# langtech-bsc/quantool

Hardware: AMD Instinct MI355X
Metric: quantized weights/sec (GPTQ int4, Llama-3-8B, 512 calib samples) (higher is better)
Workload: dtype f32

## Files before the change

### include/quantool_amd.h

```cpp
#ifndef QUANTOOL_AMD_H
#define QUANTOOL_AMD_H

#include <stddef.h>
#include <stdint.h>

#ifdef __cplusplus
extern "C" {
#endif

typedef void* qt_stream_t;

enum qt_status {
    QT_OK = 0,
    QT_ERR_INVALID = -1,
    QT_ERR_NOT_PD = -2,
    QT_ERR_WORKSPACE = -3,
    QT_ERR_HIP = -4,
    QT_ERR_UNSUPPORTED = -5
};

enum qt_dtype { QT_F32 = 0, QT_BF16 = 1, QT_F16 = 2 };

int qt_version(void);
const char* qt_last_error(void);

size_t qt_xtx_workspace_bytes(int64_t n_tokens, int K);
int qt_xtx_accumulate(const void* X, int x_dtype, int64_t n_tokens, int K, int64_t ldx, float* G,
                      void* workspace, size_t workspace_bytes, qt_stream_t stream);

int qt_xtx_accumulate_batched(const void* const* X, int x_dtype, const int64_t* n_tokens, const int64_t* ldx, int K,
                              float* const* G, int n_problems, void* workspace, size_t workspace_bytes,
                              qt_stream_t stream);
int qt_xtx_batched_plan(const int64_t* n_tokens, int n_problems, int K, int32_t* items, int max_items, int* n_items,
                        int* n_slabs, size_t* workspace_bytes);

size_t qt_xtx_accumulate_f32_workspace_bytes(int64_t n_tokens, int K);
int qt_xtx_accumulate_f32(const float* X, int64_t n_tokens, int K, int64_t ldx, float* G, void* workspace,
                          size_t workspace_bytes, qt_stream_t stream);

size_t qt_act_stats_workspace_bytes(int64_t n_tokens, int K);
int qt_act_stats_accumulate(const void* X, int x_dtype, int64_t n_tokens, int K, int64_t ldx, float* abs_sum,
                            float* cmin, float* cmax, void* workspace, size_t workspace_bytes,
                            qt_stream_t stream);

size_t qt_hessian_prepare_workspace_bytes(int K);
int qt_hessian_prepare(const float* G, int K, int64_t n_samples, float percdamp,
                       const int32_t* perm, float* A, uint8_t* dead, float* diag_out,
                       void* workspace, size_t workspace_bytes, qt_stream_t stream);
int qt_hessian_prepare_damp(const float* G, int K, int64_t n_samples, float percdamp,
                            const int32_t* perm, float* A, uint8_t* dead, float* diag_out, float* damp_out,
                            void* workspace, size_t workspace_bytes, qt_stream_t stream);
int qt_hessian_diag(const float* G, int K, int64_t n_samples, float* diag_out, qt_stream_t stream);
int qt_argsort_desc(const float* values, int K, int32_t* perm, int32_t* inv, qt_stream_t stream);

size_t qt_cholesky_inverse_upper_workspace_bytes(int K);
int qt_cholesky_inverse_upper(float* A, int K, float* U, int32_t* info, void* workspace,
                              size_t workspace_bytes, qt_stream_t stream);

size_t qt_cholesky_inverse_upper_batched_workspace_bytes(int K, int n_problems);
int qt_cholesky_inverse_upper_batched(float* A, int64_t strideA, int K, float* U, int64_t strideU, int32_t* info,
                                      int n_problems, void* workspace, size_t workspace_bytes, qt_stream_t stream);

int qt_cholesky_inverse_upper_bounded(float* A, int K, float* U, int32_t* info, const float* min_eig_lb,
                                      void* workspace, size_t workspace_bytes, qt_stream_t stream);
int qt_cholesky_inverse_upper_batched_bounded(float* A, int64_t strideA, int K, float* U, int64_t strideU, int32_t* info,
                                              int n_problems, const float* min_eig_lb, void* workspace,
                                              size_t workspace_bytes, qt_stream_t stream);

int qt_group_minmax_qparams(const void* W, int w_dtype, int R, int K, int64_t ldw, int group_size,
                            int symmetric, int num_bits, float* scale, float* zp, float* scale_t,
                            float* zp_t, qt_stream_t stream);

int qt_weight_gather_f32(const void* W, int w_dtype, int R, int K, int64_t ldw, const int32_t* perm,
                         const uint8_t* dead, float* W_f32, qt_stream_t stream);

int qt_weight_gather_qparams(const void* W, int w_dtype, int R, int K, int64_t ldw, const int32_t* perm,
                             const uint8_t* dead, int group_size, int symmetric, int num_bits, float* W_f32, float* scale,
                             float* zp, float* scale_t, float* zp_t, int64_t ld_t, qt_stream_t stream);

size_t qt_gptq_sweep_workspace_bytes(int R, int K, int blocksize);
int qt_gptq_sweep(float* W, int R, int K, const float* U, const float* scale_t, const float* zp_t,
                  int G, const int32_t* g_idx, int blocksize, int num_bits, int8_t* Qt,
                  float* loss, void* workspace, size_t workspace_bytes, qt_stream_t stream);

int qt_gptq_sweep_grouped(float* W, int R, int K, const float* U, int64_t strideU, int n_groups, const int32_t* row_end,
                          const float* scale_t, const float* zp_t, int G, const int32_t* g_idx, int blocksize,
                          int num_bits, int8_t* Qt, float* loss, void* workspace, size_t workspace_bytes,
                          qt_stream_t stream);

int qt_pack_int4(const int8_t* Qt, int R, int K, const int32_t* col_src, int32_t* packed,
                 qt_stream_t stream);

int qt_dequantize(const int8_t* Qt, int R, int K, const int32_t* col_src, const float* scale,
                  const float* zp, int G, const int32_t* g_of_col, void* out, int out_dtype,
                  int64_t ldo, qt_stream_t stream);

size_t qt_awq_weight_mean_workspace_bytes(int R, int K);
int qt_awq_weight_mean_accumulate(const void* W, int w_dtype, int R, int K, int64_t ldw, int group_size,
                                  float* w_sum, void* workspace, size_t workspace_bytes,
                                  qt_stream_t stream);
int qt_awq_scales(const float* x_abs_sum, int64_t n_tokens, const float* w_sum, int64_t n_rows, int K,
                  int n_grid, int duo_scaling, float* scales, qt_stream_t stream);
int qt_symmetrize_lower(float* G, int K, qt_stream_t stream);
size_t qt_awq_loss_workspace_bytes(int R, int K);
int qt_awq_loss(const void* W, int w_dtype, int R, int K, int64_t ldw, const float* s, int group_size,
                int symmetric, int num_bits, const float* Gfull, int64_t n_tokens, int exact, float weight,
                int accumulate, float* loss_out, void* workspace, size_t workspace_bytes, qt_stream_t stream);
size_t qt_awq_losses_workspace_bytes(int R, int K, int n_grid);
int qt_awq_losses(const void* W, int w_dtype, int R, int K, int64_t ldw, const float* scales, int n_grid,
                  int group_size, int symmetric, int num_bits, const float* Gfull, int64_t n_tokens, float weight,
                  int accumulate, float* losses, void* workspace, size_t workspace_bytes, qt_stream_t stream);
int qt_argmin_f32(const float* values, int n, int32_t* index_out, qt_stream_t stream);
int qt_awq_pseudo_quantize(const void* W, int w_dtype, int R, int K, int64_t ldw, const float* s, int group_size,
                           int symmetric, int num_bits, void* out, int64_t ldo, qt_stream_t stream);
int qt_scale_columns(const void* W, int w_dtype, int R, int K, int64_t ldw, const float* s, int divide,
                     void* out, int64_t ldo, qt_stream_t stream);
int qt_rtn_quantize(const void* W, int w_dtype, int R, int K, int64_t ldw, const float* scale,
                    const float* zp, int G, int group_size, int num_bits, int8_t* Qt, qt_stream_t stream);

size_t qt_col_absmax_workspace_bytes(int R, int K);
int qt_col_absmax_accumulate(const void* W, int w_dtype, int R, int K, int64_t ldw, float* wmax,
                             void* workspace, size_t workspace_bytes, qt_stream_t stream);
int qt_smoothquant_scales(const float* cmin, const float* cmax, const float* wmax, int K, float alpha,
                          float* s, qt_stream_t stream);

size_t qt_sgemm_tn_f32_workspace_bytes(int M, int N);
int qt_sgemm_tn_f32(const float* A, int64_t lda, const float* B, int64_t ldb, const float* Cin,
                    int64_t ldcin, float* Cout, int64_t ldcout, int M, int N, int kdim, int skip_zero_k,
                    int mode, int allow_split_k, void* workspace, size_t workspace_bytes, qt_stream_t stream);

int qt_xtx_tile_table_check(int K, int* n_tiles_out, int* chunk_panels_out, int* round_panels_out);

size_t qt_xtx_dot_workspace_bytes(int64_t n_tokens, int K);
int qt_xtx_dot(const void* X, int x_dtype, int64_t n_tokens, int K, int64_t ldx, const float* H, double scale,
               float* out, int accumulate, void* workspace, size_t workspace_bytes, qt_stream_t stream);

size_t qt_gemm3_tn_f32_workspace_bytes(int M, int N, int k);
int qt_gemm3_tn_f32(const float* A, int64_t lda, const float* B, int64_t ldb, float* C, int64_t ldc, int M,
                    int N, int k, int kind, void* workspace, size_t workspace_bytes, qt_stream_t stream);
int qt_gemm3_tn_f32_ex(const float* A, int64_t lda, const float* B, int64_t ldb, float* C, int64_t ldc, int M, int N,
                       int k, int kind, int tri, int tight, int batch, int64_t bsA, int64_t bsB, int64_t bsC,
                       void* workspace, size_t workspace_bytes, qt_stream_t stream);

int qt_gemm3_tn_f16x2(const float* A, int64_t lda, const float* B, int64_t ldb, float* C, int64_t ldc, int M, int N,
                      int k, int kind, int tri, int tight, int batch, int64_t bsA, int64_t bsB, int64_t bsC,
                      const float* bound_a, const float* bound_b, void* workspace, size_t workspace_bytes,
                      qt_stream_t stream);

int qt_gemm3_plan_check(int Tm, int Tn, int c_end, int tri, int* n_items_out, int* n_slabs_out, int* longest_out);
int qt_chol_g3_plan_check(int K, int merged, int min_chunks, long long* counts_out);
enum qt_act { QT_ACT_SILU = 0 };
#define QT_I8_MID_MAX_M 128
#define QT_I8_MID_K_UNIT 128
#define QT_I8_RING_K_UNIT 128
#define QT_I8_RING_SLOTS 8
#define QT_I8_RING_LEAD 6
#define QT_I8_RING_W4_K_UNIT 128
#define QT_I8_RING_W4_SLOTS 8
#define QT_I8_RING_W4_LEAD 6
#define QT_SPLITK_I8_K_UNIT 128
#define QT_SPLITK_I8_MAX_SPLITS 32
#define QT_SPLITK_I8_MIN_K_TILES 4
#define QT_MOE_I8_WIDE_K_UNIT 128
#define QT_MOE_I8_WIDE_TILE_ROWS 128
#define QT_MOE_I8_WIDE_MAX_E 4096
enum qt_weight_format { QT_W_INT8 = 0, QT_W_INT4_PACKED = 1 };
int qt_quantize_tokens_i8(const void* X, int x_dtype, int64_t M, int K, int64_t ldx, const int32_t* col_perm,
                          int symmetric, int8_t* Xq, float* s_x, int32_t* zp_x, qt_stream_t stream);
int qt_act_mul_quantize_i8(const void* gate, int64_t ldg, const void* up, int64_t ldu, int x_dtype, int64_t M, int K,
                           int act, const int32_t* col_perm, int symmetric, int8_t* Xq, float* s_x, int32_t* zp_x,
                           void* H, int64_t ldh, qt_stream_t stream);
int qt_rmsnorm_quantize_i8(const void* X, int64_t ldx, const void* weight, int x_dtype, int64_t M, int K, float eps,
                           const int32_t* col_perm, int symmetric, int8_t* Xq, float* s_x, int32_t* zp_x,
                           void* Y, int64_t ldy, float* rstd, qt_stream_t stream);
int qt_gemm_i8(const int8_t* Xq, int64_t M, int K, const void* Wq, int w_format, int N, const float* s_x,
               const int32_t* zp_x, const float* s_w, int G, const int32_t* wsum, const void* bias, void* Y,
               int out_dtype, int64_t ldy, qt_stream_t stream);
int qt_gemm_i8_skinny(const int8_t* Xq, int M, int K, const void* Wq, int w_format, int N, const float* s_x,
                      const int32_t* zp_x, const float* s_w, int G, const int32_t* wsum, const void* bias, void* Y,
                      int out_dtype, int64_t ldy, qt_stream_t stream);
int qt_gemm_i8_ring(const int8_t* Xq, int64_t M, int K, const void* Wq, int w_format, int N, const float* s_x,
                    const int32_t* zp_x, const float* s_w, int G, const int32_t* wsum, const void* bias, void* Y,
                    int out_dtype, int64_t ldy, qt_stream_t stream);
int qt_gemm_i8_ring_w4(const int8_t* Xq, int64_t M, int K, const void* Wq, int w_format, int N, const float* s_x,
                       const int32_t* zp_x, const float* s_w, int G, const int32_t* wsum, const void* bias, void* Y,
                       int out_dtype, int64_t ldy, qt_stream_t stream);
int qt_gemm_i8_mid(const int8_t* Xq, int64_t M, int K, const void* Wq, int w_format, int N, const float* s_x,
                   const int32_t* zp_x, const float* s_w, int G, const int32_t* wsum, const void* bias, void* Y,
                   int out_dtype, int64_t ldy, qt_stream_t stream);
int qt_splitk_gemm_i8_plan(int64_t M, int N, int K, int cus, int splits_requested, int* splits,
                           size_t* workspace_size);
int qt_splitk_gemm_i8_range(int k_tiles, int splits, int s, int* t0, int* t1);
int qt_splitk_gemm_i8(const int8_t* Xq, int64_t M, int K, const void* Wq, int w_format, int N, const float* s_x,
                      const int32_t* zp_x, const float* s_w, int G, const int32_t* wsum, const void* bias, void* Y,
                      int out_dtype, int64_t ldy, int splits, void* workspace, size_t workspace_size,
                      qt_stream_t stream);

int qt_moe_route(const void* top_k_index, int index_is_int64, int64_t T, int k, int E, int32_t* offsets,
                 int32_t* src_token, int32_t* src_slot, int32_t* row_of, qt_stream_t stream);
int qt_gemm_i8_grouped(const int8_t* Xq, int K, const int32_t* row_idx, int64_t R, const int32_t* offsets, int E,
                       const void* Wq, int w_format, int N, const float* s_x, const int32_t* zp_x, const float* s_w,
                       int G, const int32_t* wsum, void* Y, int out_dtype, int64_t ldy, qt_stream_t stream);
int qt_gemm_i8_skinny_grouped(const int8_t* Xq, int K, const int32_t* row_idx, int64_t R, const int32_t* offsets,
                              int E, const void* Wq, int w_format, int N, const float* s_x, const int32_t* zp_x,
                              const float* s_w, int G, const int32_t* wsum, void* Y, int out_dtype, int64_t ldy,
                              qt_stream_t stream);
int qt_gemm_i8_ring_grouped(const int8_t* Xq, int K, const int32_t* row_idx, int64_t R, const int32_t* offsets, int E,
                            const void* Wq, int w_format, int N, const float* s_x, const int32_t* zp_x,
                            const float* s_w, int G, const int32_t* wsum, void* Y, int out_dtype, int64_t ldy,
                            int64_t x_rows, qt_stream_t stream);
int qt_moe_gemm_i8_ring_w4(const int8_t* Xq, int K, const int32_t* row_idx, int64_t R, const int32_t* offsets, int E,
                           const void* Wq, int w_format, int N, const float* s_x, const int32_t* zp_x,
                           const float* s_w, int G, const int32_t* wsum, void* Y, int out_dtype, int64_t ldy,
                           int64_t x_rows, qt_stream_t stream);
int qt_moe_gemm_i8_wide(const int8_t* Xq, int K, const int32_t* row_idx, int64_t R, const int32_t* offsets, int E,
                        const void* Wq, int w_format, int N, const float* s_x, const int32_t* zp_x, const float* s_w,
                        int G, const int32_t* wsum, void* Y, int out_dtype, int64_t ldy, int64_t x_rows,
                        qt_stream_t stream);
int qt_moe_combine(const void* Y, int dtype, int H, int64_t ldy, const int32_t* row_of, const float* weights,
                   int64_t T, int k, void* out, qt_stream_t stream);

int qt_dequantize_weight(const void* Wq, int w_format, int N, int K, const float* s_w, int G, const int8_t* zp_w,
                         const int32_t* g_idx, void* W, int dtype, int64_t ldw, qt_stream_t stream);
int qt_gemm_wq_skinny(const void* X, int x_dtype, int M, int K, int64_t ldx, const void* Wq, int w_format, int N,
                      const float* s_w, int G, const int8_t* zp_w, const int32_t* g_idx, const void* bias, void* Y,
                      int64_t ldy, qt_stream_t stream);

int qt_gemm_wq_stream(const void* X, int x_dtype, int M, int K, int64_t ldx, const void* Wq, int w_format, int N,
                      const float* s_w, int G, const int8_t* zp_w, const int32_t* g_idx, const void* bias, void* Y,
                      int64_t ldy, qt_stream_t stream);
#define QT_WQ_STREAM_MAX_M 128
#define QT_WQ_STREAM_K_UNIT 128
#define QT_WQ_STREAM_MAX_LDX 33554432
// ... 36 lines not shown
```

### quantool_amd/csrc/cholesky.hip

```cpp
#include <stdlib.h>
#include <string.h>

#include <map>
#include <tuple>
#include <vector>

#include "chol_layout.h"
#include "common.h"
#include "gemm3_tn.h"
#include "sgemm_tn.h"

namespace {

static_assert(CHOL_CHUNK_ROWS == G3_CHUNK_ROWS, "chol_layout.h counts k chunks as gemm3_tn.h cuts them");
static int chol_block_env(const char* name) {
    const char* e = getenv(name);
    if (!e) return 0;
    int x = atoi(e) / 128 * 128;
    return x < 128 ? 128 : (x > NBO_MAX ? NBO_MAX : x);
}
struct G3Step {
    int n_items = 0, n_red = 0;
    size_t item_off = 0, red_off = 0;
};
// ... 448 lines not shown
    const int blk = blk0 + blockIdx.x;
    const int n = (K - blk * NB < NB) ? K - blk * NB : NB;
    const float* Rd = Rd_all + (size_t)blk * RD_STRIDE;
    const int tid = threadIdx.x, lane = tid & 63, wave = tid >> 6;
    {
        constexpr int NV = RD_STRIDE / 4 / 256;
        f32x4 v[NV];
#pragma unroll
        for (int r = 0; r < NV; ++r) v[r] = ((const f32x4*)Rd)[tid + 256 * r];
#pragma unroll
        for (int r = 0; r < NV; ++r) ((f32x4*)Rs)[tid + 256 * r] = v[r];
    }
    const float* D32 = Rs + NB * NB;
    const int l31 = lane & 31, h = lane >> 5;
    const int col = wave * 32 + l31;

    f32x16 acc[4];
#pragma unroll
    for (int a = 0; a < 4; ++a)
#pragma unroll
        for (int r = 0; r < 16; ++r) {
            const int row = 32 * a + (r & 3) + 8 * (r >> 2) + 4 * h;
            acc[a][r] = (row == col) ? 1.0f : 0.0f;
        }
    __syncthreads();

#pragma unroll
    for (int b = 0; b < 4; ++b) {
        f32x16 zb;
#pragma unroll
        for (int r = 0; r < 16; ++r) zb[r] = 0.0f;
#pragma unroll
        for (int r = 0; r < 16; ++r) {
            const int k = (r & 3) + 8 * (r >> 2) + 4 * h;
            const float av = D32[(b * 32 + k) * 32 + l31];
            zb = __builtin_amdgcn_mfma_f32_32x32x2f32(av, acc[b][r], zb, 0, 0, 0);
        }
        acc[b] = zb;
#pragma unroll
        for (int a = b + 1; a < 4; ++a) {
#pragma unroll
            for (int r = 0; r < 16; ++r) {
                const int k = (r & 3) + 8 * (r >> 2) + 4 * h;
                const float av = -Rs[(32 * b + k) * NB + 32 * a + l31];
                acc[a] = __builtin_amdgcn_mfma_f32_32x32x2f32(av, zb[r], acc[a], 0, 0, 0);
            }
        }
    }
    float* Dinv = Dinv_all + (size_t)blk * NB * NB;
    float* Yd = Y + (size_t)(blk * NB) * ldy + blk * NB;
#pragma unroll
    for (int a = 0; a < 4; ++a)
#pragma unroll
        for (int r = 0; r < 16; ++r) {
            const int row = 32 * a + (r & 3) + 8 * (r >> 2) + 4 * h;
            const bool in = row < n && col < n;
            const float z = (in && row >= col) ? acc[a][r] : 0.0f;
            Dinv[col * NB + row] = z;
            if (in) Yd[(size_t)row * ldy + col] = z;
        }
}

__global__ __launch_bounds__(256) void transpose_lower_block_kernel(const float* __restrict__ Y, int64_t ldy, int w,
                                                                    float* __restrict__ XT, int ldx, int64_t bsY,
                                                                    int64_t bsXT) {
    if (blockIdx.z) {
        Y += (size_t)blockIdx.z * bsY;
        XT += (size_t)blockIdx.z * bsXT;
    }
    __shared__ float tile[32][33];
    const int bx = blockIdx.x * 32, by = blockIdx.y * 32;
    const int tx = threadIdx.x & 31, ty = threadIdx.x >> 5;
    for (int r = ty; r < 32; r += 8) {
        const int m = bx + r, k = by + tx;
        tile[r][tx] = (m < w && k < w && k <= m) ? Y[(size_t)m * ldy + k] : 0.0f;
    }
    __syncthreads();
    for (int r = ty; r < 32; r += 8) {
        const int k = by + r, m = bx + tx;
        if (k < w && m < w) XT[(size_t)k * ldx + m] = tile[tx][r];
    }
}

__global__ __launch_bounds__(256) void flat_reverse_lower_to_upper_kernel(float* __restrict__ U, int K, int64_t bsU) {
    U += (size_t)blockIdx.z * bsU;
    const int j = blockIdx.x * blockDim.x + threadIdx.x;
    const int i = blockIdx.y;
    if (j >= K || j < i) return;
    const size_t e = (size_t)i * K + j;
    const size_t pe = (size_t)(K - 1 - i) * K + (K - 1 - j);
    if (i == j) {
        if (e <= pe) {
            const float t = U[e];
            U[e] = U[pe];
            U[pe] = t;
        }
    } else {
        U[e] = U[pe];
        U[pe] = 0.0f;
    }
}

__global__ __launch_bounds__(256) void identity_if_failed_kernel(float* __restrict__ U, int K,
                                                                 const int32_t* __restrict__ info, int64_t bsU) {
    if (info[blockIdx.z] == 0) return;
    U += (size_t)blockIdx.z * bsU;
    for (int i = blockIdx.x; i < K; i += gridDim.x)
        for (int j = threadIdx.x; j < K; j += blockDim.x) U[(size_t)i * K + j] = (i == j) ? 1.0f : 0.0f;
}

__global__ __launch_bounds__(256) void chol_scales_kernel(const float* __restrict__ A, int64_t bsA, int K,
                                                          const float* __restrict__ min_eig_lb, int32_t* __restrict__ e,
                                                          int32_t* __restrict__ info) {
    __shared__ float red[256];
    const int b = blockIdx.x, nprob = gridDim.x;
    const float* Ab = A + (size_t)b * bsA;
    float m = 0.0f;
    for (int i = threadIdx.x; i < K; i += 256) m = fmaxf(m, Ab[(size_t)i * K + i]);
    red[threadIdx.x] = m;
    __syncthreads();
    for (int s = 128; s > 0; s >>= 1) {
        if ((int)threadIdx.x < s) red[threadIdx.x] = fmaxf(red[threadIdx.x], red[threadIdx.x + s]);
        __syncthreads();
    }
    if (threadIdx.x == 0) {
        auto clampe = [](float t) { return (int)fminf(fmaxf(t, (float)-G3_E_MAX), (float)G3_E_MAX); };
        const float d = red[0], lb = min_eig_lb[b];
        e[b] = (d > 0.0f && d < 3.0e38f) ? clampe(3.0f - ceilf(0.5f * log2f(d))) : 0;
        if (lb > 0.0f && lb < 3.0e38f) {
            e[nprob + b] = clampe(3.0f - ceilf(-0.5f * log2f(lb)));
        } else {
            e[nprob + b] = 0;
            info[b] = K + 1;
        }
    }
}

}


static CholLayout chol_layout(int K, const CholG3Plan* g3) { return CholLayout(K, g3->any, g3->max_slabs); }

extern "C" size_t qt_cholesky_inverse_upper_batched_workspace_bytes(int K, int n_problems) {
    if (K <= 0 || n_problems <= 0) return 0;
    int nbo_, nbi_;
    const CholG3Plan* g3 = chol_blocks(K, nbo_, nbi_);
    return chol_layout(K, g3).batch_bytes(n_problems, g3->blob_bytes);
}

extern "C" size_t qt_cholesky_inverse_upper_workspace_bytes(int K) {
    return qt_cholesky_inverse_upper_batched_workspace_bytes(K, 1);
}

constexpr size_t INV_LDS = (size_t)(NB * LDT + NB * LDP) * sizeof(float);
constexpr size_t POTF2_LDS = (size_t)(NB * LDA + 4 * 32 * 32) * sizeof(float);
constexpr size_t RD_LDS = RD_STRIDE * sizeof(float);

struct CholCtx {
    float *A, *Y;
    int K, nprob, NBO, NBI;
    int64_t sA, sY, sW;
    float *T, *TI, *XT, *Rd, *Dinv, *split_ws;
    size_t split_ws_bytes;
    unsigned short *Rpl, *Ypl;
    int64_t plane_stride;
    float* g3_slabs;
    char* g3_tab;
    const CholG3Plan* g3;
    const CholG3Plan* tab;
    int planes;
    int merge_mode;
    int32_t *info, *eR, *eY;
    int prio;
    hipStream_t stream;
};

static int chol_resolve(CholCtx& c, const float* min_eig_lb) {
    bool f16x2 = min_eig_lb != nullptr;
    if (const char* e = getenv("QT_CHOL_PLANES")) {
        if (strcmp(e, "bf16x3") == 0) f16x2 = false;
        else if (strcmp(e, "f16x2") == 0) {
            QT_CHECK_ARG(min_eig_lb, "qt_cholesky_inverse_upper: QT_CHOL_PLANES=f16x2 needs a bound on lambda_min (the _bounded entry points)");
        } else {
// ... 166 lines not shown
    if (rc) return rc;
    return split_row(c, I);
}

static int chol_run_two_phase(const CholCtx& c) {
    for (BlockRow J(c.K, c.NBO); J; ++J) {
        int rc = fac_product(c, J);
        if (!rc) rc = fac_panels(c, J);
        if (rc) return rc;
    }
    int rc = trinv(c, 0, (c.K + NB - 1) / NB);
    if (rc) return rc;
    for (BlockRow I(c.K, c.NBI); I; ++I) {
        rc = inv_product(c, I);
        if (!rc) rc = inv_row(c, I);
        if (rc) return rc;
    }
    return QT_OK;
}

static int chol_run_walk(const CholCtx& c) {
    for (BlockRow J(c.K, c.NBO); J; ++J) {
        int rc;
        if (c.merge_mode == CHOL_WALK_MERGED && c.tab->row[J.Jb].n_items > 0) {
            rc = g3_row(c, c.tab->row[J.Jb], c.Rpl, J.J0, J.J0, J.rows(), c.K - J.J0, c.A + (size_t)J.J0 * c.K + J.J0, IN_A, G3_SUB,
                        true);
        } else {
            rc = fac_product(c, J);
            if (!rc) rc = inv_product(c, J);
        }
        if (!rc) rc = fac_panels(c, J);
        if (!rc) rc = trinv(c, J.J0 / NB, (J.rows() + NB - 1) / NB);
        if (!rc) rc = inv_row(c, J);
        if (rc) return rc;
    }
    return QT_OK;
}

static hipError_t chol_lds_attrs() {
    static QtOncePerDevice lds_attr;
    return lds_attr.run([] {
        const auto attr = hipFuncAttributeMaxDynamicSharedMemorySize;
        hipError_t e = hipFuncSetAttribute((const void*)potf2_kernel, attr, (int)POTF2_LDS);
        if (e == hipSuccess) e = hipFuncSetAttribute((const void*)trsm_rt_kernel, attr, (int)RD_LDS);
        if (e == hipSuccess) e = hipFuncSetAttribute((const void*)trinv_batched_kernel, attr, (int)INV_LDS);
        if (e == hipSuccess) e = hipFuncSetAttribute((const void*)trinv_mfma_kernel, attr, (int)RD_LDS);
        return e;
    });
}

static int chol_run(float* A, int64_t strideA, int K, float* U, int64_t strideU, int32_t* info, int nprob, void* workspace,
                    size_t workspace_bytes, hipStream_t stream, const float* min_eig_lb = nullptr) {
    CholCtx c = {};
    c.A = A; c.Y = U; c.K = K; c.nprob = nprob; c.info = info; c.stream = stream;
    if (int rc = chol_resolve(c, min_eig_lb)) return rc;
    const CholLayout L = chol_layout(K, c.g3);
    const size_t need = L.batch_bytes(nprob, c.g3->blob_bytes);
    if (!workspace || workspace_bytes < need) {
        qt_set_error("qt_cholesky_inverse_upper: workspace %zu < required %zu", workspace_bytes, need);
        return QT_ERR_WORKSPACE;
    }
    char* ws = (char*)qt_align_up((size_t)workspace, 256);
    c.sW = (int64_t)(L.bytes() / 4); c.sA = nprob > 1 ? strideA : 0; c.sY = nprob > 1 ? strideU : 0;
    c.T = (float*)(ws + L.T); c.TI = (float*)(ws + L.TI); c.XT = (float*)(ws + L.XT);
    c.Rd = (float*)(ws + L.Rd); c.Dinv = (float*)(ws + L.Dinv);
    c.split_ws = (float*)(ws + L.split); c.split_ws_bytes = L.split_bytes;
    c.plane_stride = (int64_t)K * K;
    if (c.g3->any) {
        c.Rpl = (unsigned short*)(ws + L.Rpl); c.Ypl = (unsigned short*)(ws + L.Ypl);
        c.g3_slabs = (float*)(ws + L.slabs); c.g3_tab = ws + L.tables(nprob);
        QT_HIP(hipMemcpyAsync(c.g3_tab, c.tab->blob, c.tab->blob_bytes, hipMemcpyHostToDevice, stream));
    }
    static_assert(2 * SG_MAX_BATCH * sizeof(int32_t) <= (size_t)NB * NB * 2, "the exponents fit the smallest third plane");
    c.eR = c.planes == G3_F16X2 ? (int32_t*)(c.Rpl + 2 * c.plane_stride) : nullptr;
    c.eY = c.planes == G3_F16X2 ? c.eR + nprob : nullptr;
    QT_HIP(chol_lds_attrs());
    QT_HIP(hipMemsetAsync(info, 0, sizeof(int32_t) * nprob, stream));
    c.prio = qt_chain_prio();
    if (c.planes == G3_F16X2) {
        hipLaunchKernelGGL(chol_scales_kernel, dim3(nprob), dim3(256), 0, stream, (const float*)A, c.sA, K, min_eig_lb, c.eR, info);
        QT_LAUNCH_CHECK();
    }
    if (int rc = c.merge_mode == CHOL_TWO_PHASE ? chol_run_two_phase(c) : chol_run_walk(c)) return rc;
    hipLaunchKernelGGL(flat_reverse_lower_to_upper_kernel, dim3((K + 255) / 256, K, nprob), dim3(256), 0, stream, U, K, c.sY);
    QT_LAUNCH_CHECK();
    hipLaunchKernelGGL(identity_if_failed_kernel, dim3(K < 1024 ? K : 1024, 1, nprob), dim3(256), 0, stream, U, K,
                       (const int32_t*)info, c.sY);
    QT_LAUNCH_CHECK();
    return QT_OK;
}

static int chol_check_batch(const char* fn, bool ptrs, int K, int n_problems, int64_t strideA, int64_t strideU) {
    QT_CHECK_ARG(K > 0 && ptrs && n_problems >= 1 && n_problems <= SG_MAX_BATCH, "%s: bad arguments (1 <= n_problems <= %d)", fn,
                 SG_MAX_BATCH);
    QT_CHECK_ARG(n_problems == 1 || (strideA >= (int64_t)K * K && strideU >= (int64_t)K * K && strideA % 4 == 0 && strideU % 4 == 0),
                 "%s: strides must be multiples of 4 elements and >= K*K", fn);
    return QT_OK;
}

extern "C" int qt_cholesky_inverse_upper(float* A, int K, float* U, int32_t* info, void* workspace,
                                         size_t workspace_bytes, qt_stream_t stream_) {
    QT_CHECK_ARG(K > 0 && A && U && info, "qt_cholesky_inverse_upper: bad arguments");
    return chol_run(A, 0, K, U, 0, info, 1, workspace, workspace_bytes, (hipStream_t)stream_);
}

extern "C" int qt_cholesky_inverse_upper_batched(float* A, int64_t strideA, int K, float* U, int64_t strideU, int32_t* info,
                                                 int n_problems, void* workspace, size_t workspace_bytes,
                                                 qt_stream_t stream_) {
    if (int rc = chol_check_batch("qt_cholesky_inverse_upper_batched", A && U && info, K, n_problems, strideA, strideU)) return rc;
    return chol_run(A, strideA, K, U, strideU, info, n_problems, workspace, workspace_bytes, (hipStream_t)stream_);
}

extern "C" int qt_cholesky_inverse_upper_bounded(float* A, int K, float* U, int32_t* info, const float* min_eig_lb,
                                                 void* workspace, size_t workspace_bytes, qt_stream_t stream_) {
    QT_CHECK_ARG(K > 0 && A && U && info && min_eig_lb, "qt_cholesky_inverse_upper_bounded: bad arguments");
    return chol_run(A, 0, K, U, 0, info, 1, workspace, workspace_bytes, (hipStream_t)stream_, min_eig_lb);
}

extern "C" int qt_cholesky_inverse_upper_batched_bounded(float* A, int64_t strideA, int K, float* U, int64_t strideU,
                                                         int32_t* info, int n_problems, const float* min_eig_lb,
                                                         void* workspace, size_t workspace_bytes, qt_stream_t stream_) {
    if (int rc = chol_check_batch("qt_cholesky_inverse_upper_batched_bounded", A && U && info && min_eig_lb, K, n_problems,
                                  strideA, strideU))
        return rc;
    return chol_run(A, strideA, K, U, strideU, info, n_problems, workspace, workspace_bytes, (hipStream_t)stream_, min_eig_lb);
}

extern "C" int qt_chol_g3_plan_check(int K, int merged, int min_chunks, long long* counts_out) {
    if (K <= 0) return -1;
    constexpr int NBX = 512, TRI_STEP = 256 / G3_CHUNK_ROWS;
    if (min_chunks <= 0) min_chunks = 64;
    const int cap = chol_g3_target_items(K);
    CholG3Plan sep, pl;
    std::vector<char> sep_bytes, bytes;
    chol_g3_build(K, NBX, NBX, min_chunks, cap, false, sep, sep_bytes);
    chol_g3_build(K, NBX, NBX, min_chunks, cap, merged != 0, pl, bytes);
    if (pl.max_slabs > sep.max_slabs || pl.blob_bytes > sep.blob_bytes) return -2;
    long long launches = 0, n_items = 0, n_slabs = 0;
    auto check = [&](const G3Step& st, int Tm, int Tn0, int tri0, int Tn1, int c_end) -> int {
        if (st.n_items <= 0) return 0;
        const G3Item* items = (const G3Item*)(bytes.data() + st.item_off);
        const G3Red* red = (const G3Red*)(bytes.data() + st.red_off);
        if (st.n_items > cap && st.n_items > Tm * (Tn0 + Tn1)) return -3;
        const int Tn[2] = {Tn0, Tn1};
        auto lo_of = [&](int seg, int tj) { return (seg == 1 || tri0) ? TRI_STEP * tj : 0; };
        std::vector<int> cover((size_t)2 * Tm * (Tn0 + Tn1 + 1) * c_end, 0);
        auto cell = [&](int seg, int ti, int tj, int c) { return (((size_t)seg * Tm + ti) * (Tn0 + Tn1 + 1) + tj) * c_end + c; };
        std::vector<int> owner(sep.max_slabs, -1);
        int slabs_here = 0;
        for (int q = 0; q < st.n_items; ++q) {
            const G3Item& it = items[q];
            const int seg = (it.tile & G3_SEG_BIT) ? 1 : 0, ti = it.tile >> 16, tj = it.tile & G3_TJ_MASK;
            if (ti < 0 || ti >= Tm || tj >= Tn[seg]) return -4;
            const int lo = lo_of(seg, tj);
            if (it.c_lo < lo || it.c_hi > c_end || it.c_hi - it.c_lo < 2) return -5;
            for (int c = it.c_lo; c < it.c_hi; ++c) cover[cell(seg, ti, tj, c)]++;
            if (it.slab < 0) {
                if (it.c_lo != lo || it.c_hi != c_end) return -6;
            } else {
                if (it.slab >= sep.max_slabs) return -7;
                if (owner[it.slab] >= 0) return -8;
                owner[it.slab] = q;
                ++slabs_here;
            }
        }
        for (int seg = 0; seg < 2; ++seg)
            for (int ti = 0; ti < Tm; ++ti)
                for (int tj = 0; tj < Tn[seg]; ++tj)
                    for (int c = 0; c < c_end; ++c)
                        if (cover[cell(seg, ti, tj, c)] != (c >= lo_of(seg, tj) ? 1 : 0)) return -9;
        int in_red = 0;
        for (int r = 0; r < st.n_red; ++r) {
            const G3Red& e = red[r];
            if (e.count < 2 || e.first < 0 || e.first + e.count > sep.max_slabs || (e.seg != 0 && e.seg != 1)) return -10;
            const int want_tile = e.tile | (e.seg ? G3_SEG_BIT : 0);
            int prev_hi = lo_of(e.seg, e.tile & G3_TJ_MASK);
            for (int q = 0; q < e.count; ++q) {
                const int o = owner[e.first + q];
                if (o < 0 || items[o].tile != want_tile || items[o].c_lo != prev_hi) return -11;
                prev_hi = items[o].c_hi;
// ... 33 lines not shown
```

### quantool_amd/csrc/quant.hip

```cpp
#include "common.h"

namespace {


__device__ __forceinline__ float wave_min(float v) {
#pragma unroll
    for (int o = 32; o > 0; o >>= 1) v = fminf(v, __shfl_xor(v, o));
    return v;
}
__device__ __forceinline__ float wave_max(float v) {
#pragma unroll
    for (int o = 32; o > 0; o >>= 1) v = fmaxf(v, __shfl_xor(v, o));
    return v;
}

__global__ __launch_bounds__(64) void qparams_kernel(const void* __restrict__ W, int dtype, int R, int K,
                                                     int64_t ldw, int gs, int symmetric, float qmin, float qmax,
                                                     float* __restrict__ scale, float* __restrict__ zp,
                                                     float* __restrict__ scale_t, float* __restrict__ zp_t) {
    const int g = blockIdx.x, r = blockIdx.y, lane = threadIdx.x;
    const int G = K / gs;
    const size_t base = (size_t)r * ldw + (size_t)g * gs;
    float mn = INFINITY, mx = -INFINITY;
    for (int c = lane; c < gs; c += 64) {
        const float w = qt_load_w(W, dtype, base + c);
        mn = fminf(mn, w);
        mx = fmaxf(mx, w);
    }
    mn = wave_min(mn);
    mx = wave_max(mx);
    if (lane == 0) {
        mn = fminf(mn, 0.0f);
        mx = fmaxf(mx, 0.0f);
        float s, z;
        const float eps = 1.1920928955078125e-07f;
        if (symmetric) {
            const float amax = fmaxf(fabsf(mn), fabsf(mx));
            s = amax / ((qmax - qmin) / 2.0f);
            s = fmaxf(s, eps);
            z = 0.0f;
        } else {
            s = (mx - mn) / (qmax - qmin);
            s = fmaxf(s, eps);
            z = qmin - mn / s;
            z = fminf(fmaxf(rintf(z), qmin), qmax);
        }
        scale[(size_t)r * G + g] = s;
        zp[(size_t)r * G + g] = z;
        if (scale_t) scale_t[(size_t)g * R + r] = s;
        if (zp_t) zp_t[(size_t)g * R + r] = z;
    }
}

__global__ __launch_bounds__(256) void gather_f32_kernel(const void* __restrict__ W, int dtype, int R, int K,
                                                         int64_t ldw, const int32_t* __restrict__ perm,
                                                         const uint8_t* __restrict__ dead, float* __restrict__ out) {
    const int s = blockIdx.x * blockDim.x + threadIdx.x;
    const int r = blockIdx.y;
    if (s >= K) return;
    const int src = perm ? perm[s] : s;
    float v = qt_load_w(W, dtype, (size_t)r * ldw + src);
    if (dead && dead[s]) v = 0.0f;
    out[(size_t)r * K + s] = v;
}

template <typename T>
__global__ __launch_bounds__(256) void gather_qparams_kernel(const T* __restrict__ W, int dtype, int R, int K, int64_t ldw,
                                                             const int32_t* __restrict__ perm,
                                                             const uint8_t* __restrict__ dead, int gs, int symmetric,
                                                             float qmin, float qmax, float* __restrict__ out,
                                                             float* __restrict__ scale, float* __restrict__ zp,
                                                             float* __restrict__ scale_t, float* __restrict__ zp_t,
                                                             int64_t ld_t) {
    extern __shared__ __attribute__((aligned(16))) unsigned char smem[];
    T* row = (T*)smem;
    const int r = blockIdx.x, tid = threadIdx.x, lane = tid & 63, wave = tid >> 6;
    const T* src = W + (size_t)r * ldw;
    constexpr int V = 16 / sizeof(T);
    if ((((uintptr_t)src) & 15) == 0 && K % V == 0) {
        for (int c = tid * V; c < K; c += 256 * V) *(f32x4*)(row + c) = *(const f32x4*)(src + c);
    } else {
        for (int c = tid; c < K; c += 256) row[c] = src[c];
// ... 41 lines not shown
            f32x4 v;
#pragma unroll
            for (int e = 0; e < 4; ++e) {
                const int sp = s4 + e;
                const float x = val(perm ? perm[sp] : sp);
                v[e] = (dead && dead[sp]) ? 0.0f : x;
            }
            *(f32x4*)(dst + s4) = v;
        }
    } else {
        for (int sp = tid; sp < K; sp += 256) {
            const float x = val(perm ? perm[sp] : sp);
            dst[sp] = (dead && dead[sp]) ? 0.0f : x;
        }
    }
}

__global__ __launch_bounds__(256) void pack_int4_kernel(const int8_t* __restrict__ Qt, int R, int K,
                                                        const int32_t* __restrict__ col_src,
                                                        int32_t* __restrict__ packed) {
    __shared__ uint32_t tile[64][33];
    const int Kw = (K + 7) / 8;
    const int r0 = blockIdx.y * 64, w0 = blockIdx.x * 32;
    const int tid = threadIdx.x;
    for (int e = tid; e < 64 * 32; e += 256) {
        const int rl = e & 63, wl = e >> 6;
        const int r = r0 + rl, w = w0 + wl;
        uint32_t acc = 0;
        if (r < R && w < Kw) {
#pragma unroll
            for (int j = 0; j < 8; ++j) {
                const int c = w * 8 + j;
                if (c < K) {
                    const int sc = col_src ? col_src[c] : c;
                    const uint32_t u = ((uint32_t)((int)Qt[(size_t)sc * R + r] + 8)) & 0xFu;
                    acc |= u << (4 * j);
                }
            }
        }
        tile[rl][wl] = acc;
    }
    __syncthreads();
    for (int e = tid; e < 64 * 32; e += 256) {
        const int wl = e & 31, rl = e >> 5;
        const int r = r0 + rl, w = w0 + wl;
        if (r < R && w < Kw) packed[(size_t)r * Kw + w] = (int32_t)tile[rl][wl];
    }
}

__global__ __launch_bounds__(256) void pack_int4_rows4_kernel(const int8_t* __restrict__ Qt, int R, int K,
                                                              const int32_t* __restrict__ col_src,
                                                              int32_t* __restrict__ packed) {
    __shared__ uint32_t tile[256][33];
    const int Kw = (K + 7) / 8;
    const int r0 = blockIdx.y * 256, w0 = blockIdx.x * 32;
    const int tid = threadIdx.x;
    for (int e = tid; e < 64 * 32; e += 256) {
        const int rq = e & 63, wl = e >> 6;
        const int r = r0 + 4 * rq, w = w0 + wl;
        uint32_t acc[4] = {0, 0, 0, 0};
        if (r < R && w < Kw) {
#pragma unroll
            for (int j = 0; j < 8; ++j) {
                const int c = w * 8 + j;
                if (c < K) {
                    const int sc = col_src ? col_src[c] : c;
                    const uint32_t q4 = *(const uint32_t*)(Qt + (size_t)sc * R + r);
#pragma unroll
                    for (int i = 0; i < 4; ++i) {
                        const uint32_t u = (uint32_t)((int)(int8_t)(q4 >> (8 * i)) + 8) & 0xFu;
                        acc[i] |= u << (4 * j);
                    }
                }
            }
        }
#pragma unroll
        for (int i = 0; i < 4; ++i) tile[4 * rq + i][wl] = acc[i];
    }
    __syncthreads();
    for (int e = tid; e < 256 * 32; e += 256) {
        const int wl = e & 31, rl = e >> 5;
        const int r = r0 + rl, w = w0 + wl;
        if (r < R && w < Kw) packed[(size_t)r * Kw + w] = (int32_t)tile[rl][wl];
    }
}

__global__ __launch_bounds__(256) void dequant_kernel(const int8_t* __restrict__ Qt, int R, int K,
                                                      const int32_t* __restrict__ col_src,
                                                      const float* __restrict__ scale, const float* __restrict__ zp,
                                                      int G, const int32_t* __restrict__ g_of_col,
                                                      void* __restrict__ out, int out_dtype, int64_t ldo) {
    __shared__ float tile[64][65];
    const int r0 = blockIdx.y * 64, c0 = blockIdx.x * 64;
    const int tid = threadIdx.x;
    for (int e = tid; e < 64 * 64; e += 256) {
        const int rl = e & 63, cl = e >> 6;
        const int r = r0 + rl, c = c0 + cl;
        float v = 0.0f;
        if (r < R && c < K) {
            const int sc = col_src ? col_src[c] : c;
            v = (float)Qt[(size_t)sc * R + r];
        }
        tile[rl][cl] = v;
    }
    __syncthreads();
    for (int e = tid; e < 64 * 64; e += 256) {
        const int cl = e & 63, rl = e >> 6;
        const int r = r0 + rl, c = c0 + cl;
        if (r < R && c < K) {
            const int g = g_of_col[c];
            const float q = tile[rl][cl];
            const float z = zp[(size_t)r * G + g];
            const float v = (q - z) * scale[(size_t)r * G + g];
            qt_store_w(out, out_dtype, (size_t)r * ldo + c, v);
        }
    }
}

}

static inline void qt_range(int num_bits, float* qmin, float* qmax) {
    *qmin = -(float)(1 << (num_bits - 1));
    *qmax = (float)((1 << (num_bits - 1)) - 1);
}

extern "C" int qt_group_minmax_qparams(const void* W, int w_dtype, int R, int K, int64_t ldw, int group_size,
                                       int symmetric, int num_bits, float* scale, float* zp, float* scale_t,
                                       float* zp_t, qt_stream_t stream_) {
    hipStream_t stream = (hipStream_t)stream_;
    QT_CHECK_ARG(W && scale && zp && R > 0 && K > 0, "qt_group_minmax_qparams: bad arguments");
    QT_CHECK_ARG(qt_dtype_ok(w_dtype), "qt_group_minmax_qparams: dtype %d unsupported", w_dtype);
    QT_CHECK_ARG(num_bits >= 2 && num_bits <= 8, "qt_group_minmax_qparams: num_bits=%d", num_bits);
    const int gs = group_size <= 0 ? K : group_size;
    QT_CHECK_ARG(K % gs == 0, "qt_group_minmax_qparams: K=%d not divisible by group_size=%d", K, gs);
    float qmin, qmax;
    qt_range(num_bits, &qmin, &qmax);
    const size_t esz = qt_dtype_size(w_dtype);
    const int G = K / gs;
    for (int row0 = 0; row0 < R; row0 += 32768) {
        const int rows = (R - row0 < 32768) ? R - row0 : 32768;
        hipLaunchKernelGGL(qparams_kernel, dim3(G, rows), dim3(64), 0, stream,
                           (const void*)((const char*)W + (size_t)row0 * ldw * esz), w_dtype, R, K, ldw, gs, symmetric,
                           qmin, qmax, scale + (size_t)row0 * G, zp + (size_t)row0 * G,
                           scale_t ? scale_t + row0 : nullptr, zp_t ? zp_t + row0 : nullptr);
        QT_LAUNCH_CHECK();
    }
    return QT_OK;
}

extern "C" int qt_weight_gather_f32(const void* W, int w_dtype, int R, int K, int64_t ldw, const int32_t* perm,
                                    const uint8_t* dead, float* W_f32, qt_stream_t stream_) {
    hipStream_t stream = (hipStream_t)stream_;
    QT_CHECK_ARG(W && W_f32 && R > 0 && K > 0, "qt_weight_gather_f32: bad arguments");
    QT_CHECK_ARG(qt_dtype_ok(w_dtype), "qt_weight_gather_f32: dtype %d unsupported", w_dtype);
    const size_t esz = qt_dtype_size(w_dtype);
    for (int row0 = 0; row0 < R; row0 += 32768) {
        const int rows = (R - row0 < 32768) ? R - row0 : 32768;
        hipLaunchKernelGGL(gather_f32_kernel, dim3((K + 255) / 256, rows), dim3(256), 0, stream,
                           (const void*)((const char*)W + (size_t)row0 * ldw * esz), w_dtype, rows, K, ldw, perm, dead,
                           W_f32 + (size_t)row0 * K);
        QT_LAUNCH_CHECK();
    }
    return QT_OK;
}

extern "C" int qt_weight_gather_qparams(const void* W, int w_dtype, int R, int K, int64_t ldw, const int32_t* perm,
                                        const uint8_t* dead, int group_size, int symmetric, int num_bits, float* W_f32,
                                        float* scale, float* zp, float* scale_t, float* zp_t, int64_t ld_t,
                                        qt_stream_t stream_) {
    hipStream_t stream = (hipStream_t)stream_;
    QT_CHECK_ARG(W && W_f32 && scale && zp && R > 0 && K > 0, "qt_weight_gather_qparams: bad arguments");
    QT_CHECK_ARG(qt_dtype_ok(w_dtype), "qt_weight_gather_qparams: dtype %d unsupported", w_dtype);
    QT_CHECK_ARG(num_bits >= 2 && num_bits <= 8, "qt_weight_gather_qparams: num_bits=%d", num_bits);
    const int gs = group_size <= 0 ? K : group_size;
    QT_CHECK_ARG(K % gs == 0, "qt_weight_gather_qparams: K=%d not divisible by group_size=%d", K, gs);
    QT_CHECK_ARG((!scale_t && !zp_t) || ld_t >= R, "qt_weight_gather_qparams: ld_t=%lld < R=%d", (long long)ld_t, R);
    const size_t esz = qt_dtype_size(w_dtype);
    const size_t lds = qt_align_up((size_t)K * esz, 16);
    QT_CHECK_ARG(lds <= 160 * 1024, "qt_weight_gather_qparams: a row of %d elements does not fit the LDS", K);
    QT_CHECK_ARG(((uintptr_t)W_f32 & 15) == 0, "qt_weight_gather_qparams: W_f32 must be 16-byte aligned");
    float qmin, qmax;
    qt_range(num_bits, &qmin, &qmax);
    static QtOncePerDevice attr16, attr32;
    if (esz == 2) {
        QT_HIP(attr16.run([&] {
            return hipFuncSetAttribute((const void*)gather_qparams_kernel<unsigned short>,
                                       hipFuncAttributeMaxDynamicSharedMemorySize, 160 * 1024);
        }));
        hipLaunchKernelGGL(gather_qparams_kernel<unsigned short>, dim3(R), dim3(256), lds, stream, (const unsigned short*)W,
                           w_dtype, R, K, ldw, perm, dead, gs, symmetric, qmin, qmax, W_f32, scale, zp, scale_t, zp_t, ld_t);
    } else {
        QT_HIP(attr32.run([&] {
            return hipFuncSetAttribute((const void*)gather_qparams_kernel<float>, hipFuncAttributeMaxDynamicSharedMemorySize,
                                       160 * 1024);
        }));
        hipLaunchKernelGGL(gather_qparams_kernel<float>, dim3(R), dim3(256), lds, stream, (const float*)W, w_dtype, R, K, ldw,
                           perm, dead, gs, symmetric, qmin, qmax, W_f32, scale, zp, scale_t, zp_t, ld_t);
    }
    QT_LAUNCH_CHECK();
    return QT_OK;
}

extern "C" int qt_pack_int4(const int8_t* Qt, int R, int K, const int32_t* col_src, int32_t* packed,
                            qt_stream_t stream_) {
    hipStream_t stream = (hipStream_t)stream_;
    QT_CHECK_ARG(Qt && packed && R > 0 && K > 0, "qt_pack_int4: bad arguments");
    const int Kw = (K + 7) / 8;
    if (R % 4 == 0 && (((uintptr_t)Qt) & 3) == 0 && (R + 255) / 256 <= 65535)
        hipLaunchKernelGGL(pack_int4_rows4_kernel, dim3((Kw + 31) / 32, (R + 255) / 256), dim3(256), 0, stream, Qt, R, K,
                           col_src, packed);
    else
        hipLaunchKernelGGL(pack_int4_kernel, dim3((Kw + 31) / 32, (R + 63) / 64), dim3(256), 0, stream, Qt, R, K, col_src,
                           packed);
    QT_LAUNCH_CHECK();
    return QT_OK;
}

extern "C" int qt_dequantize(const int8_t* Qt, int R, int K, const int32_t* col_src, const float* scale,
                             const float* zp, int G, const int32_t* g_of_col, void* out, int out_dtype, int64_t ldo,
                             qt_stream_t stream_) {
    hipStream_t stream = (hipStream_t)stream_;
    QT_CHECK_ARG(Qt && scale && zp && g_of_col && out && R > 0 && K > 0 && G > 0, "qt_dequantize: bad arguments");
    QT_CHECK_ARG(qt_dtype_ok(out_dtype), "qt_dequantize: dtype %d unsupported", out_dtype);
    hipLaunchKernelGGL(dequant_kernel, dim3((K + 63) / 64, (R + 63) / 64), dim3(256), 0, stream, Qt, R, K, col_src,
                       scale, zp, G, g_of_col, out, out_dtype, ldo);
    QT_LAUNCH_CHECK();
    return QT_OK;
}
```

### quantool_amd/csrc/xtx.hip

```cpp
#include <stdlib.h>
#include <string.h>

#include <algorithm>
#include <map>
#include <type_traits>
#include <vector>

#include "common.h"
#include "ring_pipe.h"

namespace {

constexpr int BKT = 64;
constexpr int RING = 8;

struct XtxParams {
    const void* X;
    const void* tail;
    int64_t ldx;
    int K;
    int n_tt;
    int has_tail;
    const int* tile_tab;
    int n_direct;
    int n_rem;
    int s2;
    float* slabs;
    float* G;
    int map_mode;
    int wrap_units;
    unsigned* progress;
    int thr_win;
    int thr_nap;
    int thr_chk;
    const float* H;
    double* dot_partials;
    int batch_items;
    int64_t x_batch_bytes;
    const struct XtxBItem* b_items;
    const struct XtxBProb* b_probs;
};

struct XtxBItem {
    int prob;
    int tile;
    int tt0, cnt;
    int slab;
    int pad[3];
};
struct XtxBProb {
    const void* X;
    const void* tail;
    float* G;
    int64_t ldx;
    int n_tt, has_tail;
    int64_t pad[3];
};
struct XtxBRed {
    int prob, tile, slab0, n_chunks, stride;
    int pad[3];
};
static_assert(sizeof(XtxBItem) == 32 && sizeof(XtxBProb) == 64 && sizeof(XtxBRed) == 32, "table records");

__device__ __forceinline__ int xtx_uni(int v) { return __builtin_amdgcn_readfirstlane(v); }
__device__ __forceinline__ uint64_t xtx_uni64(uint64_t v) {
    const unsigned lo = (unsigned)__builtin_amdgcn_readfirstlane((int)(unsigned)v);
    const unsigned hi = (unsigned)__builtin_amdgcn_readfirstlane((int)(unsigned)(v >> 32));
    return ((uint64_t)hi << 32) | lo;
}

__device__ __forceinline__ int xtx_logical(int map_mode) {
    const int b = blockIdx.x, nwg = gridDim.x;
    if (map_mode != 0) return b;
    const int round = b >> 8, rb = b & 255;
    const int m = min(256, nwg - (round << 8));
    const int xcd = rb & 7, idx = rb >> 3, q8 = m >> 3, r8 = m & 7;
    return (round << 8) + (xcd < r8 ? xcd * (q8 + 1) : r8 * (q8 + 1) + (xcd - r8) * q8) + idx;
}

__device__ __forceinline__ int xtx_item(const XtxParams& p, int logical, int& tt0, int& cnt, int& slab_idx) {
    int tile_idx;
    slab_idx = -1;
    if (logical < p.n_direct) {
        tile_idx = logical;
        tt0 = 0;
        cnt = p.n_tt;
    } else {
        const int l2 = logical - p.n_direct;
        const int chunk = l2 / p.n_rem;
        tile_idx = p.n_direct + (l2 - chunk * p.n_rem);
        const int base_cnt = p.n_tt / p.s2, rem = p.n_tt % p.s2;
        tt0 = chunk * base_cnt + (chunk < rem ? chunk : rem);
        cnt = base_cnt + (chunk < rem ? 1 : 0);
        slab_idx = l2;
    }
    return p.tile_tab[tile_idx];
}


template <bool WRAP, bool F16, bool THROTTLE>
__global__ __launch_bounds__(NTHREADS, 2) void xtx_kernel(XtxParams p) {
    constexpr int LEAD = 6;
    __shared__ __attribute__((aligned(16))) char ring[RING * UNIT_BYTES + (THROTTLE ? 1024 : 0)];
    const int tid = threadIdx.x;
    const int lane = tid & 63;
    const int wave = __builtin_amdgcn_readfirstlane(tid >> 6);
    const int wave_m = wave >> 2, wave_n = wave & 3;
    const bool group_b = wave >= 4;

    const int logical = xtx_logical(p.map_mode);
    int tt0, cnt, slab_idx;
    const int tt_packed = xtx_item(p, logical, tt0, cnt, slab_idx);
    const int ti = tt_packed >> 16, tj = tt_packed & 0xFFFF;
    const int nu = cnt * (BKT / UT);
    const int K = p.K;
    const size_t ld2 = (size_t)p.ldx * 2;

    const int rsub = lane >> 4;
    const int lch = (lane & 15) ^ (rsub << 2);
    const int trow = 4 * (wave & 3) + rsub;
    int colA = ti * BT + (wave >> 2) * 128 + lch * 8;
    int colB = tj * BT + (wave >> 2) * 128 + lch * 8;
    colA = colA > K - 8 ? K - 8 : colA;
    colB = colB > K - 8 ? K - 8 : colB;
// ... 73 lines not shown
    const int rowpart = (8 * (g >> 1) + q) * 256 + 32 * (g & 1) + 8 * pp;
    int aoff[4], boff[2];
#pragma unroll
    for (int mi = 0; mi < 4; ++mi) aoff[mi] = wave_m * 4096 + rowpart + 64 * (mi ^ q);
#pragma unroll
    for (int ni = 0; ni < 2; ++ni)
        boff[ni] = (2 + (wave_n >> 1)) * 4096 + rowpart + 64 * ((((wave_n & 1) << 1) + ni) ^ q);

    f32x16 acc[4][2];
#pragma unroll
    for (int mi = 0; mi < 4; ++mi)
#pragma unroll
        for (int ni = 0; ni < 2; ++ni)
#pragma unroll
            for (int r = 0; r < 16; ++r) acc[mi][ni][r] = 0.0f;

    s16x8 fa[4], fb[2];
    auto drain_wait = [&](int u) {
        ring_drain_wait<2, LEAD>(nu - u - 2);
    };
    auto phase = [&](auto slot_c, auto steady_c, int u) {
        constexpr int S = decltype(slot_c)::value;
        constexpr bool STEADY = decltype(steady_c)::value;
        constexpr int ISLOT = (S + LEAD) & (RING - 1);
        const char* base = ring + S * UNIT_BYTES;
#pragma unroll
        for (int mi = 0; mi < 4; ++mi) fa[mi] = tr_load8(base + aoff[mi]);
#ifdef QT_XTX_ABL_LDS
        fb[0] = tr_load8(base + boff[0]);
        fb[1] = fb[0];
#else
#pragma unroll
        for (int ni = 0; ni < 2; ++ni) fb[ni] = tr_load8(base + boff[ni]);
#endif
        if (STEADY) {
            issue_running(ISLOT);
            wait_vmcnt<2 * (LEAD - 1)>();
        } else if (u + LEAD < nu) {
            issue(u + LEAD, ISLOT);
            wait_vmcnt<2 * (LEAD - 1)>();
        } else {
            drain_wait(u);
        }
#ifdef QT_XTX_ABL_HALF
        constexpr int MI_N = 2;
#else
        constexpr int MI_N = 4;
#endif
        ring_sync_math([&] { ring_mma32<F16, MI_N>(fa, fb, acc); });
    };
    auto body8 = [&](auto steady_c, int u) {
        if (THROTTLE && throttled && (u & (p.thr_chk - 1)) == 0) throttle_step(u);
        ring_body<8>([&](auto slot_c, int uu) { phase(slot_c, steady_c, uu); }, u);
    };

    if (nu > 0) {
#pragma unroll
        for (int i = 0; i < LEAD; ++i)
            if (i < nu) issue(i, i);
        if (nu >= LEAD) wait_vmcnt<2 * (LEAD - 1)>();
        else wait_vmcnt<0>();
        ring_stagger_begin(group_b);

        const int steady_end = (nu < i_tail ? nu : i_tail);
        run_src += (size_t)LEAD * ustride;
        int u = 0;
        for (; u + 8 + LEAD <= steady_end; u += 8) body8(std::true_type{}, u);
        for (; u + 8 <= nu; u += 8) body8(std::false_type{}, u);
        if (u < nu) {
            phase(std::integral_constant<int, 0>{}, std::false_type{}, u);
            phase(std::integral_constant<int, 1>{}, std::false_type{}, u + 1);
            phase(std::integral_constant<int, 2>{}, std::false_type{}, u + 2);
            phase(std::integral_constant<int, 3>{}, std::false_type{}, u + 3);
        }
        ring_stagger_end(group_b);
        if (THROTTLE && throttled && lane == 0) {
            unsigned* dst = prog_round + prog_member;
            const unsigned val = 0x7fffffffu;
            asm volatile("global_store_dword %0, %1, off sc0 sc1\n\ts_nop 1" ::"v"(dst), "v"(val) : "memory");
        }
    }

    const int jl = lane & 31, ih = 4 * (lane >> 5);
    if (slab_idx < 0) {
#pragma unroll
        for (int mi = 0; mi < 4; ++mi)
#pragma unroll
            for (int ni = 0; ni < 2; ++ni) {
                const int gj = tj * BT + wave_n * 64 + ni * 32 + jl;
#pragma unroll
                for (int r = 0; r < 16; ++r) {
                    const int gi = ti * BT + wave_m * 128 + mi * 32 + (r & 3) + 8 * (r >> 2) + ih;
                    if (gi < K && gj < K) {
                        float* dst = p.G + (size_t)gi * K + gj;
                        *dst = *dst + acc[mi][ni][r];
                    }
                }
            }
    } else {
        float* slab = p.slabs + (size_t)slab_idx * (size_t)(BT * BT);
#pragma unroll
        for (int mi = 0; mi < 4; ++mi)
#pragma unroll
            for (int ni = 0; ni < 2; ++ni)
#pragma unroll
                for (int r = 0; r < 16; ++r) {
                    const int i_loc = wave_m * 128 + mi * 32 + (r & 3) + 8 * (r >> 2) + ih;
                    const int j_loc = wave_n * 64 + ni * 32 + jl;
                    slab[i_loc * BT + j_loc] = acc[mi][ni][r];
                }
    }
}

constexpr int RING16 = 10;
constexpr int DBL_BYTES = 2 * UNIT_BYTES;

template <bool F16, bool DOT = false, bool BATCHED = false>
__global__ __launch_bounds__(NTHREADS, 2) void xtx16_kernel(XtxParams p) {
    static_assert(!(DOT && BATCHED), "the fused product has its own batch form");
    constexpr int ND = 5;
    constexpr int LEAD = 3;
    __shared__ __attribute__((aligned(16))) char ring[RING16 * UNIT_BYTES];
    const int tid = threadIdx.x;
    const int lane = tid & 63;
    const int wave = __builtin_amdgcn_readfirstlane(tid >> 6);
    const int wave_m = wave >> 2, wave_n = wave & 3;
    const bool group_b = wave >= 4;

    int logical = xtx_logical(p.map_mode);
    const int item_global = logical;
    const char* Xb = (const char*)p.X;
    if (DOT) {
        const int prob = logical / p.batch_items;
        logical -= prob * p.batch_items;
        Xb += (size_t)prob * (size_t)p.x_batch_bytes;
    }
    int tt0, cnt, slab_idx, tt_packed;
    const void* tailp = p.tail;
    float* Gp = p.G;
    int64_t ldx = p.ldx;
    int n_tt = p.n_tt, has_tail = p.has_tail;
    if (BATCHED) {
        const XtxBItem* it = p.b_items + logical;
        const XtxBProb* pr = p.b_probs + xtx_uni(it->prob);
        tt_packed = xtx_uni(it->tile);
        tt0 = xtx_uni(it->tt0);
        cnt = xtx_uni(it->cnt);
        slab_idx = xtx_uni(it->slab);
        Xb = (const char*)xtx_uni64((uint64_t)pr->X);
        tailp = (const void*)xtx_uni64((uint64_t)pr->tail);
        Gp = (float*)xtx_uni64((uint64_t)pr->G);
        ldx = (int64_t)xtx_uni64((uint64_t)pr->ldx);
        n_tt = xtx_uni(pr->n_tt);
        has_tail = xtx_uni(pr->has_tail);
    } else {
        tt_packed = xtx_item(p, logical, tt0, cnt, slab_idx);
    }
    const int ti = tt_packed >> 16, tj = tt_packed & 0xFFFF;
    const int nd = cnt * (BKT / (2 * UT));
    const int K = p.K;
    const size_t ld2 = (size_t)ldx * 2;

    const int rsub = lane >> 4;
    const int row_hi = (wave & 3) >> 1;
    const int lch = (lane & 15) ^ (rsub << 2) ^ (row_hi << 1);
    const int trow = 4 * (wave & 3) + rsub;
    int colA = ti * BT + (wave >> 2) * 128 + lch * 8;
// ... 36 lines not shown
        for (int bj = 0; bj < 4; ++bj)
#pragma unroll
            for (int r = 0; r < 4; ++r) acc[ai][bj][r] = 0.0f;

    s16x8 fa[8], fb[4];
    auto drain_wait = [&](int d) {
        ring_drain_wait<4, LEAD>(nd - d - 2);
    };
    auto phase = [&](auto slot_c, auto steady_c, int d) {
        constexpr int S = decltype(slot_c)::value;
        constexpr bool STEADY = decltype(steady_c)::value;
        constexpr int ISLOT = (S + LEAD) % ND;
        const char* base = ring + S * DBL_BYTES;
#pragma unroll
        for (int ai = 0; ai < 8; ++ai) fa[ai] = tr_load8(base + aoff[ai]);
#pragma unroll
        for (int bj = 0; bj < 4; ++bj) fb[bj] = tr_load8(base + boff[bj]);
        if (STEADY) {
            issue_at(run_src, ISLOT);
            run_src += 2 * ustride;
            wait_vmcnt<4 * (LEAD - 1)>();
        } else if (d + LEAD < nd) {
            issue_at(dbl_src(d + LEAD), ISLOT);
            wait_vmcnt<4 * (LEAD - 1)>();
        } else {
            drain_wait(d);
        }
        ring_sync_math([&] { ring_mma16<F16>(fa, fb, acc); });
    };

    if (nd > 0) {
#pragma unroll
        for (int i = 0; i < LEAD; ++i)
            if (i < nd) issue_at(dbl_src(i), i);
        if (nd >= LEAD) wait_vmcnt<4 * (LEAD - 1)>();
        else wait_vmcnt<0>();
        ring_stagger_begin(group_b);

        const int steady_end = (nd < d_tail ? nd : d_tail);
        run_src += (size_t)LEAD * 2 * ustride;
        int d = 0;
        for (; d + ND + LEAD <= steady_end; d += ND)
            ring_body<ND>([&](auto slot_c, int dd) { phase(slot_c, std::true_type{}, dd); }, d);
        for (; d < nd; d += ND) {
            phase(std::integral_constant<int, 0>{}, std::false_type{}, d);
            if (d + 1 < nd) phase(std::integral_constant<int, 1>{}, std::false_type{}, d + 1);
            if (d + 2 < nd) phase(std::integral_constant<int, 2>{}, std::false_type{}, d + 2);
            if (d + 3 < nd) phase(std::integral_constant<int, 3>{}, std::false_type{}, d + 3);
            if (d + 4 < nd) phase(std::integral_constant<int, 4>{}, std::false_type{}, d + 4);
        }
        ring_stagger_end(group_b);
    }

    const int jl = lane & 15, ih = 4 * (lane >> 4);
    if (DOT) {
        double part = 0.0;
#pragma unroll
        for (int ai = 0; ai < 8; ++ai)
#pragma unroll
            for (int bj = 0; bj < 4; ++bj) {
                const int gj = tj * BT + wave_n * 64 + bj * 16 + jl;
#pragma unroll
                for (int r = 0; r < 4; ++r) {
                    const int gi = ti * BT + wave_m * 128 + ai * 16 + ih + r;
                    if (gi < K && gj <= gi) {
                        const double v = (double)p.H[(size_t)gi * K + gj] * (double)acc[ai][bj][r];
                        part += (gj < gi) ? 2.0 * v : v;
                    }
                }
            }
#pragma unroll
        for (int off = 32; off > 0; off >>= 1) part += __shfl_xor(part, off);
        double* red = (double*)ring;
        if (lane == 0) red[wave] = part;
        __syncthreads();
        if (tid == 0) {
            double t = red[0];
#pragma unroll
            for (int w = 1; w < 8; ++w) t += red[w];
            p.dot_partials[item_global] = t;
        }
        return;
    }
    if (slab_idx < 0) {
#pragma unroll
        for (int ai = 0; ai < 8; ++ai)
#pragma unroll
            for (int bj = 0; bj < 4; ++bj) {
                const int gj = tj * BT + wave_n * 64 + bj * 16 + jl;
#pragma unroll
                for (int r = 0; r < 4; ++r) {
                    const int gi = ti * BT + wave_m * 128 + ai * 16 + ih + r;
                    if (gi < K && gj < K) {
                        float* dst = Gp + (size_t)gi * K + gj;
                        *dst = *dst + acc[ai][bj][r];
                    }
                }
            }
    } else {
        float* slab = p.slabs + (size_t)slab_idx * (size_t)(BT * BT);
#pragma unroll
        for (int ai = 0; ai < 8; ++ai)
#pragma unroll
            for (int bj = 0; bj < 4; ++bj)
#pragma unroll
                for (int r = 0; r < 4; ++r) {
                    const int i_loc = wave_m * 128 + ai * 16 + ih + r;
                    const int j_loc = wave_n * 64 + bj * 16 + jl;
                    slab[i_loc * BT + j_loc] = acc[ai][bj][r];
                }
    }
}

__global__ __launch_bounds__(256) void xtx_reduce_kernel(const float* __restrict__ slabs, int n_rem, int n_splits,
                                                         float* __restrict__ G, int K,
                                                         const int* __restrict__ tile_tab) {
    const int tile = blockIdx.x;
    const int tt_packed = tile_tab[tile];
    const int ti = tt_packed >> 16, tj = tt_packed & 0xFFFF;
    const int part = blockIdx.y;
    const size_t tile_elems = (size_t)BT * BT;
    for (int e = threadIdx.x; e < 16 * (BT / 4); e += blockDim.x) {
        const int i_loc = part * 16 + e / (BT / 4);
        const int j_loc = (e % (BT / 4)) * 4;
        const int gi = ti * BT + i_loc, gj = tj * BT + j_loc;
        if (gi >= K || gj >= K) continue;
        f32x4 s = {0.f, 0.f, 0.f, 0.f};
        for (int sp = 0; sp < n_splits; ++sp) {
            const f32x4 v = *(const f32x4*)(slabs + ((size_t)sp * n_rem + tile) * tile_elems +
                                            (size_t)i_loc * BT + j_loc);
            s += v;
        }
        float* dst = G + (size_t)gi * K + gj;
        if (gj + 3 < K) {
            f32x4 o = *(f32x4*)dst;
            o += s;
            *(f32x4*)dst = o;
        } else {
            for (int c = 0; c < 4 && gj + c < K; ++c) dst[c] += s[c];
        }
    }
}

struct XtxPlan {
    int n_tiles, n_tt, has_tail;
    int n_direct, n_rem, s2;
    size_t slab_bytes, tail_bytes, tab_bytes, prog_bytes;
};

static void xtx_tile_order_pairs(int nt, std::vector<int>& tab) {
    const int m = 8, nb = (nt + m - 1) / m;
    auto blk = [&](int a, int b) {
        const int r0 = a * m, r1 = std::min(nt, r0 + m), c0 = b * m, c1 = std::min(nt, c0 + m);
        if (a == b) {
            for (int ti = r0; ti < r1; ++ti)
                for (int tj = c0; tj <= ti; ++tj) tab.push_back((ti << 16) | tj);
        } else {
            for (int si = r0; si < r1; si += 4)
                for (int ti = si; ti < std::min(si + 4, r1); ++ti)
                    for (int tj = c0; tj < c1; ++tj) tab.push_back((ti << 16) | tj);
        }
    };
    for (int a = 0; a < nb; a += 2) {
        if (a + 1 < nb) {
            for (int b = 0; b <= a + 1; ++b) {
                if (b <= a) blk(a, b);
                blk(a + 1, b);
            }
        } else {
            for (int b = 0; b <= a; ++b) blk(a, b);
        }
    }
}

static void xtx_tile_order_aligned(int nt, std::vector<int>& tab) {
    const int m = 8, nb = (nt + m - 1) / m;
    const bool ragged = nt % m != 0;
    const int nfull = ragged ? nb - 1 : nb;
    std::vector<int> left;
    auto blk = [&](int a, int b) {
        const int r0 = a * m, r1 = std::min(nt, r0 + m), c0 = b * m, c1 = std::min(nt, c0 + m);
        for (int si = r0; si < r1; si += 4)
            for (int ti = si; ti < std::min(si + 4, r1); ++ti)
                for (int tj = c0; tj < c1; ++tj) tab.push_back((ti << 16) | tj);
    };
    auto tri = [&](int a) {
        const int r0 = a * m, r1 = std::min(nt, r0 + m);
        const bool full = r1 - r0 == m;
        int n = 0;
        for (int ti = r0; ti < r1; ++ti)
            for (int tj = r0; tj <= ti; ++tj, ++n) (full && n < 32 ? tab : left).push_back((ti << 16) | tj);
    };
    for (int a = 0; a < nfull; a += 2) {
        if (a + 1 < nfull) {
            for (int b = 0; b < a; ++b) {
                blk(a, b);
                blk(a + 1, b);
            }
            blk(a + 1, a);
            tri(a);
            tri(a + 1);
        } else {
            for (int b = 0; b < a; ++b) blk(a, b);
            tri(a);
        }
    }
    if (ragged) {
        for (int b = 0; b < nb - 1; ++b) blk(nb - 1, b);
        tri(nb - 1);
    }
    tab.insert(tab.end(), left.begin(), left.end());
}

static int xtx_order_mode(int nt) {
    const char* e = getenv("QT_XTX_ORDER");
    const int mode = e ? atoi(e) : (nt * (nt + 1) / 2 >= NUM_CU ? 2 : 1);
    return mode < 0 || mode > 2 ? 2 : mode;
// ... 31 lines not shown
        const size_t slab_cap = (size_t)1 << 30;
        double best_cost = 1.0;
        for (int S = 2; S <= 64; ++S) {
            if (pl.n_tt / S < 4) break;
            if ((size_t)S * rem * BT * BT * 4 > slab_cap) break;
            const long wgs = (long)rem * S;
            const double cost = (double)((wgs + NUM_CU - 1) / NUM_CU) / S;
            if (cost < best_cost * 0.97) {
                best_cost = cost;
                best = S;
            }
        }
    }
    pl.s2 = best;
    if (pl.s2 == 1) {
        pl.n_direct = pl.n_tiles;
        pl.n_rem = 0;
    } else {
        pl.n_direct = n_full;
        pl.n_rem = rem;
    }
    pl.slab_bytes = (size_t)pl.s2 * pl.n_rem * BT * BT * 4;
    pl.tail_bytes = pl.has_tail ? qt_align_up((size_t)BKT * K * 2, 256) : 0;
    pl.tab_bytes = qt_align_up((size_t)pl.n_tiles * 4, 256);
    pl.prog_bytes = qt_align_up((size_t)((pl.n_tiles + NUM_CU - 1) / NUM_CU) * 256 * sizeof(unsigned), 256);
    return pl;
}

const int* xtx_host_table(int K, int n_tiles) {
    static std::mutex m;
    static std::map<std::pair<int, int>, int*> tabs;
    std::lock_guard<std::mutex> lock(m);
    const std::pair<int, int> key(K, xtx_order_mode((K + BT - 1) / BT));
    auto it = tabs.find(key);
    if (it != tabs.end()) return it->second;
    std::vector<int> v;
    xtx_tile_order((K + BT - 1) / BT, v);
    if ((int)v.size() != n_tiles) return nullptr;
    int* pinned = nullptr;
    if (hipHostMalloc((void**)&pinned, v.size() * sizeof(int), hipHostMallocDefault) != hipSuccess) return nullptr;
    for (size_t i = 0; i < v.size(); ++i) pinned[i] = v[i];
    tabs[key] = pinned;
    return pinned;
}

}

extern "C" int qt_xtx_tile_table_check(int K, int* n_tiles_out, int* chunk_panels_out, int* round_panels_out) {
    if (K <= 0) return QT_ERR_INVALID;
    const int nt = (K + BT - 1) / BT;
    std::vector<int> tab;
    xtx_tile_order(nt, tab);
    if ((long)tab.size() != (long)nt * (nt + 1) / 2) return -2;
    std::vector<char> seen((size_t)nt * nt, 0);
    for (int e : tab) {
        const int ti = e >> 16, tj = e & 0xFFFF;
        if (ti >= nt || tj > ti) return -3;
        if (seen[(size_t)ti * nt + tj]++) return -4;
    }
    auto panels = [&](int size) {
        int total = 0;
        std::vector<int> mark(nt, -1);
        for (size_t c = 0; c < tab.size(); c += size)
            for (size_t i = c; i < std::min(tab.size(), c + size); ++i)
                for (int x : {tab[i] >> 16, tab[i] & 0xFFFF})
                    if (mark[x] != (int)(c / size)) {
                        mark[x] = (int)(c / size);
                        ++total;
                    }
        return total;
    };
    if (n_tiles_out) *n_tiles_out = (int)tab.size();
    if (chunk_panels_out) *chunk_panels_out = panels(32);
    if (round_panels_out) *round_panels_out = panels(NUM_CU);
    return 0;
}

extern "C" size_t qt_xtx_workspace_bytes(int64_t n_tokens, int K) {
    if (n_tokens <= 0 || K <= 0) return 0;
    XtxPlan pl = xtx_plan(n_tokens, K);
    return pl.slab_bytes + pl.tail_bytes + pl.tab_bytes + pl.prog_bytes + 256;
}

extern "C" int qt_xtx_accumulate(const void* X, int x_dtype, int64_t n_tokens, int K, int64_t ldx, float* G,
                                 void* workspace, size_t workspace_bytes, qt_stream_t stream_) {
    hipStream_t stream = (hipStream_t)stream_;
    QT_CHECK_ARG(qt_dtype_is16(x_dtype), "qt_xtx_accumulate: x_dtype %d must be QT_BF16 or QT_F16", x_dtype);
    QT_CHECK_ARG(K > 0 && K % 8 == 0, "qt_xtx_accumulate: K=%d must be a positive multiple of 8", K);
    QT_CHECK_ARG(ldx >= K && ldx % 8 == 0, "qt_xtx_accumulate: ldx=%lld must be >= K and a multiple of 8", (long long)ldx);
    QT_CHECK_ARG(n_tokens >= 0, "qt_xtx_accumulate: n_tokens < 0");
    if (n_tokens == 0) return QT_OK;
    QT_CHECK_ARG(X && G, "qt_xtx_accumulate: null pointer");
    QT_CHECK_ARG(((uintptr_t)X & 15) == 0 && ((uintptr_t)G & 15) == 0, "qt_xtx_accumulate: X and G must be 16-byte aligned");
    QT_CHECK_ARG((uint64_t)ldx * 2 * UT + (uint64_t)K * 2 < ((uint64_t)1 << 32), "qt_xtx_accumulate: ldx too large");
    XtxPlan pl = xtx_plan(n_tokens, K);
    const size_t need = pl.slab_bytes + pl.tail_bytes + pl.tab_bytes + pl.prog_bytes + 256;
    if (workspace_bytes < need || !workspace) {
        qt_set_error("qt_xtx_accumulate: workspace %zu < required %zu", workspace_bytes, need);
        return QT_ERR_WORKSPACE;
    }
    char* ws = (char*)qt_align_up((size_t)workspace, 256);
    float* slabs = (float*)ws;
    void* tail = pl.has_tail ? (void*)(ws + pl.slab_bytes) : nullptr;
    int* tile_tab = (int*)(ws + pl.slab_bytes + pl.tail_bytes);
    const int* host_tab = xtx_host_table(K, pl.n_tiles);
    if (!host_tab) {
        qt_set_error("qt_xtx_accumulate: could not build the tile table for K=%d", K);
        return QT_ERR_HIP;
    }
    QT_HIP(hipMemcpyAsync(tile_tab, host_tab, (size_t)pl.n_tiles * 4, hipMemcpyHostToDevice, stream));
    XtxParams p;
    p.X = X;
    p.tail = tail;
    p.ldx = ldx;
    p.K = K;
    p.n_tt = pl.n_tt;
    p.has_tail = pl.has_tail;
    p.tile_tab = tile_tab;
    p.n_direct = pl.n_direct;
    p.n_rem = pl.n_rem;
    p.s2 = pl.s2;
    p.slabs = slabs;
    p.G = G;
    {
        const char* e = getenv("QT_XTX_MAP");
        p.map_mode = e ? atoi(e) : 0;
    }
    p.progress = nullptr;
    p.thr_win = 128;
    p.thr_nap = 127;
    p.thr_chk = 32;
    p.H = nullptr;
    p.dot_partials = nullptr;
    p.batch_items = 1;
    p.x_batch_bytes = 0;
    p.wrap_units = 0;
#ifdef QT_XTX_ABLATION
    {
        const char* e = getenv("QT_XTX_ABLATE_WRAP");
        p.wrap_units = e ? atoi(e) : 0;
    }
#endif
    if (pl.has_tail) {
        const int64_t full = n_tokens / BKT * BKT;
        const int64_t tail_rows = n_tokens - full;
        QT_HIP(hipMemsetAsync(tail, 0, (size_t)BKT * K * 2, stream));
        QT_HIP(hipMemcpy2DAsync(tail, (size_t)K * 2, (const char*)X + (size_t)full * ldx * 2, (size_t)ldx * 2,
                                (size_t)K * 2, (size_t)tail_rows, hipMemcpyDeviceToDevice, stream));
    }
    const char* thr_env = getenv("QT_XTX_THROTTLE");
    const bool throttle_on = thr_env ? atoi(thr_env) != 0 : true;
    unsigned* progress_ws = (unsigned*)(ws + pl.slab_bytes + pl.tail_bytes + pl.tab_bytes);
    auto launch = [&](const XtxParams& q, const XtxPlan& ql) -> int {
        const int grid = ql.n_direct + ql.n_rem * ql.s2;
        qt_prof_mark(QT_PROF_XTX, stream);
        XtxParams qq = q;
        const bool thr = throttle_on && ql.n_direct >= 4 * NUM_CU && q.n_tt >= 512 &&
                         (size_t)q.n_tt * BKT * (size_t)q.K * 2 > ((size_t)1 << 30);
        if (thr) {
            const size_t rounds = (size_t)(ql.n_direct + NUM_CU - 1) / NUM_CU;
            if (hipMemsetAsync(progress_ws, 0, rounds * 256 * sizeof(unsigned), stream) != hipSuccess) {
                qt_set_error("qt_xtx_accumulate: hipMemsetAsync(progress) failed");
                return QT_ERR_HIP;
            }
            qq.progress = progress_ws;
            static const int win = [] { const char* e = getenv("QT_XTX_THR_WIN"); return e ? atoi(e) : 128; }();
            static const int nap = [] { const char* e = getenv("QT_XTX_THR_NAP"); return e ? atoi(e) : 127; }();
            qq.thr_win = win;
            qq.thr_nap = nap;
            static const int chk = [] { const char* e = getenv("QT_XTX_THR_CHK"); const int v = e ? atoi(e) : 32; return (v == 8 || v == 16 || v == 64 || v == 128 || v == 256) ? v : 32; }();
            qq.thr_chk = chk;
        } else {
            qq.progress = nullptr;
        }
        const char* she = getenv("QT_XTX_SHAPE");
        const bool shape16 = she ? atoi(she) == 16 : !thr;
        if (shape16 && q.wrap_units == 0) {
            qq.progress = nullptr;
            if (x_dtype == QT_F16) hipLaunchKernelGGL((xtx16_kernel<true>), dim3(grid), dim3(NTHREADS), 0, stream, qq);
            else hipLaunchKernelGGL((xtx16_kernel<false>), dim3(grid), dim3(NTHREADS), 0, stream, qq);
        }
#ifdef QT_XTX_ABLATION
        else if (q.wrap_units > 0) hipLaunchKernelGGL((xtx_kernel<true, false, false>), dim3(grid), dim3(NTHREADS), 0, stream, qq);
#endif
        else if (thr && x_dtype == QT_F16) hipLaunchKernelGGL((xtx_kernel<false, true, true>), dim3(grid), dim3(NTHREADS), 0, stream, qq);
        else if (thr) hipLaunchKernelGGL((xtx_kernel<false, false, true>), dim3(grid), dim3(NTHREADS), 0, stream, qq);
        else if (x_dtype == QT_F16) hipLaunchKernelGGL((xtx_kernel<false, true, false>), dim3(grid), dim3(NTHREADS), 0, stream, qq);
        else hipLaunchKernelGGL((xtx_kernel<false, false, false>), dim3(grid), dim3(NTHREADS), 0, stream, qq);
        qt_prof_mark(QT_PROF_XTX, stream);
        QT_LAUNCH_CHECK();
        if (ql.n_rem > 0) {
            hipLaunchKernelGGL(xtx_reduce_kernel, dim3(ql.n_rem, 16), dim3(256), 0, stream, q.slabs, ql.n_rem, ql.s2,
                               q.G, q.K, q.tile_tab + ql.n_direct);
            QT_LAUNCH_CHECK();
        }
        return QT_OK;
    };
    if (pl.has_tail && ldx != K) {
        const int64_t full = n_tokens / BKT * BKT;
        if (full > 0) {
            XtxPlan pf = xtx_plan(full, K);
            if (pf.slab_bytes > pl.slab_bytes) {
                pf.s2 = 1;
                pf.n_direct = pf.n_tiles;
                pf.n_rem = 0;
                pf.slab_bytes = 0;
            }
            XtxParams pfp = p;
            pfp.n_tt = pf.n_tt;
            pfp.has_tail = 0;
            pfp.n_direct = pf.n_direct;
            pfp.n_rem = pf.n_rem;
            pfp.s2 = pf.s2;
            const int rc = launch(pfp, pf);
            if (rc != QT_OK) return rc;
        }
        XtxPlan pt = xtx_plan(BKT, K);
        pt.s2 = 1;
        pt.n_direct = pt.n_tiles;
        pt.n_rem = 0;
        XtxParams ptp = p;
        ptp.X = tail;
        ptp.ldx = K;
        ptp.n_tt = 1;
        ptp.has_tail = 0;
        ptp.n_direct = pt.n_direct;
        ptp.n_rem = 0;
        ptp.s2 = 1;
        return launch(ptp, pt);
    }
    return launch(p, pl);
}

namespace {

__global__ __launch_bounds__(256) void xtx_reduce_batched_kernel(const float* __restrict__ slabs,
                                                                 const XtxBRed* __restrict__ reds,
                                                                 const XtxBProb* __restrict__ probs, int K) {
    const XtxBRed* rd = reds + blockIdx.x;
    const int tt_packed = xtx_uni(rd->tile), slab0 = xtx_uni(rd->slab0), n_chunks = xtx_uni(rd->n_chunks),
              stride = xtx_uni(rd->stride);
    float* G = (float*)xtx_uni64((uint64_t)probs[xtx_uni(rd->prob)].G);
    const int ti = tt_packed >> 16, tj = tt_packed & 0xFFFF;
    const int part = blockIdx.y;
    const size_t tile_elems = (size_t)BT * BT;
    for (int e = threadIdx.x; e < 16 * (BT / 4); e += blockDim.x) {
        const int i_loc = part * 16 + e / (BT / 4);
        const int j_loc = (e % (BT / 4)) * 4;
        const int gi = ti * BT + i_loc, gj = tj * BT + j_loc;
        if (gi >= K || gj >= K) continue;
        f32x4 s = {0.f, 0.f, 0.f, 0.f};
        for (int c = 0; c < n_chunks; ++c) {
            const f32x4 v = *(const f32x4*)(slabs + ((size_t)slab0 + (size_t)c * stride) * tile_elems +
                                            (size_t)i_loc * BT + j_loc);
            s += v;
        }
        float* dst = G + (size_t)gi * K + gj;
        if (gj + 3 < K) {
            f32x4 o = *(f32x4*)dst;
            o += s;
            *(f32x4*)dst = o;
        } else {
            for (int c = 0; c < 4 && gj + c < K; ++c) dst[c] += s[c];
        }
    }
}

constexpr int XTX_BATCH_MAX = 16;
constexpr int XTX_MIN_CHUNK = 4;

struct XtxBPlan {
    int single = -1;
    std::vector<XtxBItem> items;
    std::vector<XtxBRed> reds;
    int n_slabs = 0, n_ragged = 0;
    int tail_slot[XTX_BATCH_MAX];
    size_t slab_bytes = 0, tail_bytes = 0, tail_stride = 0, tab_bytes = 0;
    size_t item_off = 0, prob_off = 0, red_off = 0;
    size_t need = 0;
};

int xtx_chunks_for(int n_tt, int L) { return std::max(1, std::min((n_tt + L - 1) / L, n_tt / XTX_MIN_CHUNK)); }

int xtx_batched_plan(const int64_t* n_tokens, int n_problems, int K, XtxBPlan& pl) {
    const int nt = (K + BT - 1) / BT;
    const int n_tiles = nt * (nt + 1) / 2;
    std::vector<int> tab;
    xtx_tile_order(nt, tab);
    if ((int)tab.size() != n_tiles) return QT_ERR_INVALID;
    std::vector<int> act;
    int n_tt[XTX_BATCH_MAX];
    for (int p = 0; p < n_problems; ++p) {
        n_tt[p] = (int)((n_tokens[p] + BKT - 1) / BKT);
        pl.tail_slot[p] = -1;
        if (n_tokens[p] > 0) act.push_back(p);
        if (n_tokens[p] % BKT != 0) pl.tail_slot[p] = pl.n_ragged++;
    }
    if (act.empty()) return QT_OK;
    auto emit = [&](int p, int c, int t_lo, int t_hi) {
        if (t_lo >= t_hi) return;
        const int base_cnt = n_tt[p] / c, rem = n_tt[p] % c, width = t_hi - t_lo;
        const int slab_base = pl.n_slabs;
        for (int ch = 0; ch < c; ++ch)
            for (int t = t_lo; t < t_hi; ++t) {
                XtxBItem it = {};
                it.prob = p;
                it.tile = tab[t];
                it.tt0 = ch * base_cnt + std::min(ch, rem);
                it.cnt = base_cnt + (ch < rem ? 1 : 0);
                it.slab = c > 1 ? pl.n_slabs++ : -1;
                pl.items.push_back(it);
            }
        if (c > 1)
            for (int t = t_lo; t < t_hi; ++t) {
// ... 214 lines not shown
    partials += (size_t)blockIdx.x * n;
    double acc = 0.0;
    for (int i = threadIdx.x; i < n; i += 256) acc += partials[i];
    red[threadIdx.x] = acc;
    __syncthreads();
    for (int sft = 128; sft > 0; sft >>= 1) {
        if ((int)threadIdx.x < sft) red[threadIdx.x] += red[threadIdx.x + sft];
        __syncthreads();
    }
    if (threadIdx.x == 0) {
        const float v = (float)(red[0] * scale);
        out[blockIdx.x] = accumulate ? out[blockIdx.x] + v : v;
    }
}
}

static XtxPlan xtx_frobenius_plan(int64_t n_tokens, int K, int n_batch) {
    XtxPlan pl = xtx_plan(n_tokens, K);
    if ((int64_t)pl.n_tiles * n_batch >= 4 * NUM_CU) {
        pl.n_direct = pl.n_tiles;
        pl.n_rem = 0;
        pl.s2 = 1;
    }
    return pl;
}

size_t qt_xtx_frobenius_workspace_bytes(int64_t n_tokens, int K, int n_batch) {
    if (n_tokens <= 0 || K <= 0 || n_batch <= 0) return 0;
    XtxPlan pl = xtx_frobenius_plan(n_tokens, K, n_batch);
    const size_t grid = ((size_t)pl.n_direct + (size_t)pl.n_rem * pl.s2) * n_batch;
    return pl.tab_bytes + qt_align_up(grid * sizeof(double), 256) + 256;
}

int qt_xtx_frobenius(const void* X, int x_dtype, int64_t n_tokens, int K, int64_t ldx, const float* H, double scale,
                     float* loss_out, int accumulate, void* workspace, size_t workspace_bytes, hipStream_t stream,
                     int n_batch, int64_t x_batch_stride) {
    if (!qt_dtype_is16(x_dtype) || K <= 0 || K % 8 != 0 || ldx != K || n_tokens <= 0 || n_tokens % BKT != 0 ||
        ((uintptr_t)X & 15) != 0 || (uint64_t)ldx * 2 * UT + (uint64_t)K * 2 >= ((uint64_t)1 << 32) || n_batch <= 0 ||
        (n_batch > 1 && (x_batch_stride * 2) % 16 != 0))
        return QT_ERR_UNSUPPORTED;
    XtxPlan pl = xtx_frobenius_plan(n_tokens, K, n_batch);
    const int items = pl.n_direct + pl.n_rem * pl.s2;
    if ((int64_t)items * n_batch > (int64_t)1 << 30) return QT_ERR_UNSUPPORTED;
    const size_t need = qt_xtx_frobenius_workspace_bytes(n_tokens, K, n_batch);
    if (!workspace || workspace_bytes < need) {
        qt_set_error("qt_xtx_frobenius: workspace %zu < required %zu", workspace_bytes, need);
        return QT_ERR_WORKSPACE;
    }
    char* ws = (char*)qt_align_up((size_t)workspace, 256);
    int* tile_tab = (int*)ws;
    double* partials = (double*)(ws + pl.tab_bytes);
    const int* host_tab = xtx_host_table(K, pl.n_tiles);
    if (!host_tab) {
        qt_set_error("qt_xtx_frobenius: could not build the tile table for K=%d", K);
        return QT_ERR_HIP;
    }
    QT_HIP(hipMemcpyAsync(tile_tab, host_tab, (size_t)pl.n_tiles * 4, hipMemcpyHostToDevice, stream));
    XtxParams p;
    p.X = X;
    p.tail = nullptr;
    p.ldx = ldx;
    p.K = K;
    p.n_tt = pl.n_tt;
    p.has_tail = 0;
    p.tile_tab = tile_tab;
    p.n_direct = pl.n_direct;
    p.n_rem = pl.n_rem;
    p.s2 = pl.s2;
    p.slabs = nullptr;
    p.G = nullptr;
    {
        const char* e = getenv("QT_XTX_MAP");
        p.map_mode = e ? atoi(e) : 0;
    }
    p.wrap_units = 0;
    p.progress = nullptr;
    p.thr_win = 128;
    p.thr_nap = 127;
    p.thr_chk = 32;
    p.H = H;
    p.dot_partials = partials;
    p.batch_items = items;
    p.x_batch_bytes = x_batch_stride * 2;
    const int grid = items * n_batch;
    qt_prof_mark(QT_PROF_XTX, stream);
    if (x_dtype == QT_F16) hipLaunchKernelGGL((xtx16_kernel<true, true>), dim3(grid), dim3(NTHREADS), 0, stream, p);
    else hipLaunchKernelGGL((xtx16_kernel<false, true>), dim3(grid), dim3(NTHREADS), 0, stream, p);
    qt_prof_mark(QT_PROF_XTX, stream);
    QT_LAUNCH_CHECK();
    hipLaunchKernelGGL(sum_partials_kernel, dim3(n_batch), dim3(256), 0, stream, (const double*)partials, items, scale,
                       loss_out, accumulate);
    QT_LAUNCH_CHECK();
    return QT_OK;
}

extern "C" size_t qt_xtx_dot_workspace_bytes(int64_t n_tokens, int K) { return qt_xtx_frobenius_workspace_bytes(n_tokens, K, 1); }

extern "C" int qt_xtx_dot(const void* X, int x_dtype, int64_t n_tokens, int K, int64_t ldx, const float* H, double scale,
                          float* out, int accumulate, void* workspace, size_t workspace_bytes, qt_stream_t stream) {
    QT_CHECK_ARG(X && H && out, "qt_xtx_dot: null pointer");
    const int rc = qt_xtx_frobenius(X, x_dtype, n_tokens, K, ldx, H, scale, out, accumulate, workspace, workspace_bytes,
                                    (hipStream_t)stream, 1, 0);
    if (rc == QT_ERR_UNSUPPORTED)
        qt_set_error("qt_xtx_dot: needs 16-bit X, ldx == K, K %% 8 == 0 and n_tokens %% 64 == 0 (got K=%d ldx=%lld n=%lld)", K,
                     (long long)ldx, (long long)n_tokens);
    return rc;
}
```

### quantool_amd/engine/gptq_linear.py

```python
from __future__ import annotations

from dataclasses import dataclass, field
from typing import List, Optional, Sequence, Tuple

import torch

from ..hip import ops
from .schemes import QuantArgs


class HessianAccumulator:

    STAGE_BYTES = 1 << 30
    DIRECT_TOKENS = 16384

    def __init__(self, K: int, device, stage_tokens: Optional[int] = None, dtype: Optional[torch.dtype] = None):
        self.K = K
        self.dtype = dtype
        self._G = torch.zeros((K, K), dtype=torch.float32, device=device)
        self.n = 0
        if stage_tokens is None:
            stage_tokens = max(4096, min(65536, self.STAGE_BYTES // (2 * K)))
        self.stage_tokens = int(stage_tokens) // 64 * 64
        self._stage: Optional[torch.Tensor] = None
        self._stage_sized = False
        self._fill = 0
        self._staged_on = None
        self._flushed = None

    @property
    def G(self) -> torch.Tensor:
        self.flush()
        self._after_flush()
        return self._G

    def _after_flush(self) -> None:
        if self._flushed is not None:
            stream, event = self._flushed
            here = torch.cuda.current_stream(self._G.device)
            if here != stream:
                here.wait_event(event)

    @G.setter
    def G(self, value: torch.Tensor) -> None:
        self._G = value

    def add(self, X: torch.Tensor, num_samples: Optional[int] = None) -> None:
        if num_samples is None:
            num_samples = X.shape[0] if X.dim() == 3 else 1
        X2 = X.reshape(-1, self.K)
        t = X2.shape[0]
        if X2.dtype not in (torch.bfloat16, torch.float16):
            if ops.wide_gram_mode() == "exact" and self.dtype in (None, torch.float32):
                if X2.dtype != torch.float32:
                    X2 = X2.float()
                self.dtype = torch.float32
            else:
                ops.wide_activation_policy(X2.dtype)
        self.n += int(num_samples)
        if t == 0:
            return
        if self.dtype is None:
            self.dtype = X2.dtype if X2.dtype in (torch.bfloat16, torch.float16) else torch.bfloat16
        if self.dtype == torch.float32 and not self._stage_sized:
            self._stage_sized = True
            if self.stage_tokens > 0:
                self.stage_tokens = max(128, self.stage_tokens // 2 // 128 * 128)
        if self.stage_tokens <= 0 or t >= min(self.DIRECT_TOKENS, self.stage_tokens):
            self._gram(X2 if X2.dtype == self.dtype else X2.to(self.dtype))
            return
        if self._stage is None:
            self._stage = torch.empty((self.stage_tokens, self.K), dtype=self.dtype, device=self._G.device)
        if self._fill + t > self.stage_tokens:
            self.flush()
        self._after_flush()
        self._stage[self._fill:self._fill + t].copy_(X2)
        self._fill += t
        if self._G.is_cuda:
            self._staged_on = torch.cuda.current_stream(self._G.device)

    def _gram(self, rows: torch.Tensor) -> None:
        self._after_flush()
        limit = _launch_token_limit()
        if limit <= 0 or rows.shape[0] <= limit:
            chunks = [rows]
        else:
            chunks = [rows[t0:t0 + limit] for t0 in range(0, rows.shape[0], limit)]
        for part in chunks:
            if part.dtype == torch.float32:
                ops.xtx_accumulate_f32(part, self._G)
            else:
                ops.xtx_accumulate(part, self._G)

    def flush(self) -> None:
        if self._fill:
            here = torch.cuda.current_stream(self._G.device) if self._G.is_cuda else None
            if here is not None and self._staged_on is not None and here != self._staged_on:
                here.wait_stream(self._staged_on)
            self._gram(self._stage[:self._fill])
            self._fill = 0
            self._staged_on = None
            if here is not None:
                self._flushed = (here, here.record_event())

    @staticmethod
    def flush_many(accs) -> None:
        accs = list(accs)
        groups: dict = {}
        if batched_flush_enabled():
            limit = _launch_token_limit()
            for acc in accs:
                if isinstance(acc, HessianAccumulator) and acc._fill and acc.dtype in (torch.bfloat16, torch.float16):
                    groups.setdefault((acc.K, acc.dtype, acc._G.device), []).append(acc)
            groups = {k: g for k, g in groups.items()
                      if len(g) > 1 and not (limit > 0 and any(a._fill > limit for a in g))}
        together = {id(a) for g in groups.values() for a in g}
        for acc in accs:
            if id(acc) not in together:
                acc.flush()
        for (_, _, device), group in groups.items():
            here = torch.cuda.current_stream(device) if device.type == "cuda" else None
            for b0 in range(0, len(group), ops.XTX_BATCH_MAX):
                run = group[b0:b0 + ops.XTX_BATCH_MAX]
                if len(run) == 1:
                    run[0].flush()
                    continue
                for acc in run:
                    if here is not None and acc._staged_on is not None and here != acc._staged_on:
                        here.wait_stream(acc._staged_on)
                    acc._after_flush()
                ops.xtx_accumulate_batched([acc._stage[:acc._fill] for acc in run], [acc._G for acc in run])
                event = here.record_event() if here is not None else None
                for acc in run:
                    acc._fill = 0
                    acc._staged_on = None
                    if here is not None:
                        acc._flushed = (here, event)

    def release_stage(self) -> None:
        self.flush()
        self._stage = None

    def reset(self) -> None:
        self._after_flush()
        self._fill = 0
        self._staged_on = self._flushed = None
        self._G.zero_()
        self.n = 0


flush_accumulators = HessianAccumulator.flush_many


def batched_flush_enabled() -> bool:
    import os

    return os.environ.get("QT_XTX_BATCHED", "0") == "1"


def _launch_token_limit() -> int:
    import os

    try:
        return max(0, int(os.environ.get("QT_XTX_LAUNCH_TOKENS", "0") or 0)) // 64 * 64
    except ValueError:
        return 0


def _on_device(*tensors):
    dev = torch.device("cuda", torch.cuda.current_device())
    return tuple(None if t is None else t.to(dev) for t in tensors)


@dataclass
class GPTQResult:
    weight_packed: Optional[torch.Tensor]
    weight_q: Optional[torch.Tensor]
    weight_scale: torch.Tensor
    weight_zero_point: Optional[torch.Tensor]
    weight_g_idx: Optional[torch.Tensor]
    weight_shape: torch.Tensor
    loss: torch.Tensor
    info: torch.Tensor
    scale_f32: torch.Tensor = field(repr=False, default=None)
    zp_f32: torch.Tensor = field(repr=False, default=None)
    Qt: torch.Tensor = field(repr=False, default=None)
    col_src: Optional[torch.Tensor] = field(repr=False, default=None)
    g_of_col: torch.Tensor = field(repr=False, default=None)

    def dequantized(self, dtype=torch.float32) -> torch.Tensor:
        if self.Qt is None:
            raise RuntimeError("the integer levels of this result were released (sequential driver, "
                               "QT_RESULT_DETAIL_BYTES): the module's weight holds the dequantised values")
        if self.Qt.device.type == "cpu":
            return ops.dequantize(*_on_device(self.Qt, self.scale_f32, self.zp_f32, self.g_of_col, self.col_src), dtype).cpu()
        return ops.dequantize(self.Qt, self.scale_f32, self.zp_f32, self.g_of_col, self.col_src, dtype)


def _normalize_actorder(actorder) -> Optional[str]:
    if actorder is None or actorder is False:
        return None
    a = str(actorder).lower()
    if a in ("static", "weight"):
        return "static"
    if a == "group":
        return "group"
    if a in ("none", "false"):
        return None
    raise ValueError(f"unknown actorder {actorder!r} (expected None, 'static'/'weight' or 'group')")


def gptq_quantize_shared(weights: Sequence[torch.Tensor], acc: HessianAccumulator, qargs: QuantArgs, *,
                         block_size: int = 128, dampening_frac: float = 0.01,
                         scale_dtype: Optional[torch.dtype] = None,
                         keep: Optional[dict] = None) -> List[GPTQResult]:
    return gptq_quantize_batched([(weights, acc)], qargs, block_size=block_size, dampening_frac=dampening_frac,
                                 scale_dtype=scale_dtype, keeps=None if keep is None else [keep])[0]


def batch_chains_enabled() -> bool:
    import os

    return os.environ.get("QT_BATCH_CHAINS", "1") != "0"


def batchable(groups: Sequence[Tuple[Sequence[torch.Tensor], HessianAccumulator]]) -> List[List[int]]:
    by_k = {}
    for i, (ws, acc) in enumerate(groups):
        by_k.setdefault(acc.K, []).append(i)
    out = []
    for K, idx in by_k.items():
        aligned = [i for i in idx if sum(int(w.shape[0]) for w in groups[i][0]) % 128 == 0]
        ragged = [i for i in idx if i not in aligned]
        while aligned or ragged:
            take = aligned[:ops.MAX_BATCH - 1] if ragged else aligned[:ops.MAX_BATCH]
            aligned = aligned[len(take):]
            if ragged and len(take) < ops.MAX_BATCH:
                take.append(ragged.pop(0))
            out.append(take)
    return out


def gptq_quantize_batched(groups: Sequence[Tuple[Sequence[torch.Tensor], HessianAccumulator]], qargs: QuantArgs, *,
                          block_size: int = 128, dampening_frac: float = 0.01,
                          scale_dtype: Optional[torch.dtype] = None,
                          keeps: Optional[List[dict]] = None) -> List[List[GPTQResult]]:
    n = len(groups)
    if n == 0:
        return []
    if int(block_size) != 128:
        raise ValueError(f"block_size={block_size}: this backend implements upstream's default block_size=128 only")
    K = groups[0][1].K
    dev = groups[0][1].G.device
    for ws, acc in groups:
        if acc.n <= 0:
            raise ValueError("no calibration samples were accumulated for this Linear")
        if acc.K != K:
            raise ValueError(f"batched groups must share in_features ({acc.K} != {K})")
        for w in ws:
            if w.dim() != 2 or w.shape[1] != K:
                raise ValueError(f"weight shape {tuple(w.shape)} does not match in_features {K}")
    if n > ops.MAX_BATCH:
        raise ValueError(f"at most {ops.MAX_BATCH} groups per batch (see batchable())")
    actorder = _normalize_actorder(qargs.actorder)
    gs = qargs.kernel_group_size
    gsz = K if gs <= 0 else gs
    if K % gsz:
        raise ValueError(f"in_features {K} not divisible by group_size {gsz}")
    G = K // gsz
    rows = [[int(w.shape[0]) for w in ws] for ws, _ in groups]
    grp_rows = [sum(r) for r in rows]
    if any(r % 128 for r in grp_rows[:-1]):
        raise ValueError(f"stacked groups of {grp_rows} rows: every group but the last needs a multiple of 128 (batchable())")
    R = sum(grp_rows)
    row_end = [sum(grp_rows[:i + 1]) for i in range(n)]
    row_begin = [0] + row_end[:-1]
    ar = torch.arange(K, dtype=torch.int32, device=dev)
    g_orig = (ar // gsz).to(torch.int32)

    ubuf = torch.empty((n, K * K + 256), dtype=torch.float32, device=dev)
    U = ubuf[:, :K * K].view(n, K, K)
    A = torch.empty((n, K, K), dtype=torch.float32, device=dev)
    perms, invs, deads = [], [], []
    damps = torch.zeros(n, dtype=torch.float32, device=dev) if dampening_frac > 0 else None
    for b, (ws, acc) in enumerate(groups):
        perm = inv = None
        if actorder is not None:
            perm, inv = ops.argsort_desc(ops.hessian_diag(acc.G, acc.n))
        _, dead, _ = ops.hessian_prepare(acc.G, acc.n, dampening_frac, perm, A_out=A[b], scratch=ubuf[b],
                                         damp_out=None if damps is None else damps[b:b + 1])
        perms.append(perm)
        invs.append(inv)
        deads.append(dead)

    lb = None if damps is None else torch.where(damps > 0, damps * 0.5, torch.ones_like(damps))
    if n == 1:
        _, info = ops.cholesky_inverse_upper(A[0], U_out=U[0], min_eig_lb=lb)
    else:
        info = ops.cholesky_inverse_upper_batched(A, U, min_eig_lb=lb)
    del A

    Wf = torch.empty((R, K), dtype=torch.float32, device=dev)
    g_sweeps = []
    if actorder == "group":
        for b, (ws, acc) in enumerate(groups):
            r0 = row_begin[b]
            for w, r in zip(ws, rows[b]):
                ops.weight_gather_f32(w if w.stride(1) == 1 else w.contiguous(), perms[b], deads[b], out=Wf[r0:r0 + r])
                r0 += r
            g_sweeps.append(g_orig)
        scale, zp, scale_t, zp_t = ops.group_minmax_qparams(Wf, gs, qargs.symmetric, qargs.num_bits)
    else:
        scale = torch.empty((R, G), dtype=torch.float32, device=dev)
        zp = torch.empty((R, G), dtype=torch.float32, device=dev)
        scale_t = torch.empty((G, R), dtype=torch.float32, device=dev)
        zp_t = torch.empty((G, R), dtype=torch.float32, device=dev)
        for b, (ws, acc) in enumerate(groups):
            r0 = row_begin[b]
            for w, r in zip(ws, rows[b]):
                w = w if w.stride(1) == 1 else w.contiguous()
                if K * w.element_size() <= 160 * 1024:
                    ops.weight_gather_qparams(w, perms[b], deads[b], gs, qargs.symmetric, qargs.num_bits, out=Wf[r0:r0 + r],
                                              scale=scale[r0:r0 + r], zp=zp[r0:r0 + r], scale_t=scale_t[:, r0:r0 + r],
                                              zp_t=zp_t[:, r0:r0 + r])
                else:
                    ops.weight_gather_f32(w, perms[b], deads[b], out=Wf[r0:r0 + r])
                    s_, z_, st_, zt_ = ops.group_minmax_qparams(w, gs, qargs.symmetric, qargs.num_bits)
                    scale[r0:r0 + r], zp[r0:r0 + r] = s_, z_
                    scale_t[:, r0:r0 + r], zp_t[:, r0:r0 + r] = st_, zt_
                r0 += r
            g_sweeps.append(g_orig if perms[b] is None else g_orig[perms[b].long()].contiguous())

    if keeps is not None:
        for b in range(n):
            keeps[b].update(U=U[b].clone(), perm=perms[b], dead=deads[b])
    if n == 1:
        Qt, loss = ops.gptq_sweep(Wf, U[0], scale_t, zp_t, g_sweeps[0], block_size, qargs.num_bits)
    else:
        Qt, loss = ops.gptq_sweep_grouped(Wf, U, row_end, scale_t, zp_t, torch.stack(g_sweeps).contiguous(), block_size,
                                          qargs.num_bits)
    del Wf, U, ubuf

    results: List[List[GPTQResult]] = []
    for b, (ws, acc) in enumerate(groups):
        col_src = invs[b]
        if actorder == "group":
            g_of_col = g_sweeps[b][invs[b].long()].contiguous()
        else:
            g_of_col = g_orig
        out: List[GPTQResult] = []
        r0 = row_begin[b]
        for w, r in zip(ws, rows[b]):
            Qt_i = Qt[:, r0:r0 + r].contiguous() if R > r else Qt
            sdt = scale_dtype or (w.dtype if w.dtype in (torch.bfloat16, torch.float16) else torch.float32)
            sc_i = scale[r0:r0 + r].contiguous()
            zp_i = zp[r0:r0 + r].contiguous()
            packed = ops.pack_int4(Qt_i, col_src) if qargs.num_bits == 4 else None
            wq = None
            if packed is None:
                wq = (Qt_i.t() if col_src is None else Qt_i[col_src.long()].t()).contiguous()
            out.append(GPTQResult(
                weight_packed=packed, weight_q=wq, weight_scale=sc_i.to(sdt),
                weight_zero_point=None if qargs.symmetric else zp_i.to(torch.int8),
                weight_g_idx=g_of_col if actorder == "group" else None,
                weight_shape=torch.tensor([r, K], dtype=torch.int64), loss=loss[r0:r0 + r], info=info[b:b + 1],
                scale_f32=sc_i, zp_f32=zp_i, Qt=Qt_i, col_src=col_src, g_of_col=g_of_col))
            r0 += r
        results.append(out)
    return results


def gptq_quantize_linear(weight: torch.Tensor, acc: HessianAccumulator, qargs: QuantArgs, **kw) -> GPTQResult:
    return gptq_quantize_shared([weight], acc, qargs, **kw)[0]
```

### quantool_amd/hip/_lib.py

```python
from __future__ import annotations

import ctypes
from ctypes import c_char_p, c_double, c_float, c_int, c_int32, c_int64, c_size_t, c_void_p
from pathlib import Path

_PKG = Path(__file__).resolve().parent.parent
LIB_PATH = _PKG / "lib" / "libquantool_hip.so"

QT_OK = 0
QT_ERR_INVALID = -1
QT_ERR_NOT_PD = -2
QT_ERR_WORKSPACE = -3
QT_ERR_HIP = -4
QT_ERR_UNSUPPORTED = -5

QT_F32, QT_BF16, QT_F16 = 0, 1, 2
QT_W_INT8, QT_W_INT4_PACKED = 0, 1

SIGNATURES = {
    "qt_version": (c_int, []),
    "qt_last_error": (c_char_p, []),
    "qt_xtx_workspace_bytes": (c_size_t, [c_int64, c_int]),
    "qt_xtx_accumulate": (c_int, [c_void_p, c_int, c_int64, c_int, c_int64, c_void_p, c_void_p, c_size_t, c_void_p]),
    "qt_xtx_accumulate_batched": (c_int, [c_void_p, c_int, c_void_p, c_void_p, c_int, c_void_p, c_int, c_void_p, c_size_t,
                                          c_void_p]),
    "qt_xtx_batched_plan": (c_int, [c_void_p, c_int, c_int, c_void_p, c_int, c_void_p, c_void_p, c_void_p]),
    "qt_xtx_accumulate_f32_workspace_bytes": (c_size_t, [c_int64, c_int]),
    "qt_xtx_accumulate_f32": (c_int, [c_void_p, c_int64, c_int, c_int64, c_void_p, c_void_p, c_size_t, c_void_p]),
    "qt_act_stats_workspace_bytes": (c_size_t, [c_int64, c_int]),
    "qt_act_stats_accumulate": (c_int, [c_void_p, c_int, c_int64, c_int, c_int64, c_void_p, c_void_p, c_void_p,
                                        c_void_p, c_size_t, c_void_p]),
    "qt_hessian_prepare_workspace_bytes": (c_size_t, [c_int]),
    "qt_hessian_prepare": (c_int, [c_void_p, c_int, c_int64, c_float, c_void_p, c_void_p, c_void_p, c_void_p,
                                   c_void_p, c_size_t, c_void_p]),
    "qt_hessian_prepare_damp": (c_int, [c_void_p, c_int, c_int64, c_float, c_void_p, c_void_p, c_void_p, c_void_p,
                                        c_void_p, c_void_p, c_size_t, c_void_p]),
    "qt_hessian_diag": (c_int, [c_void_p, c_int, c_int64, c_void_p, c_void_p]),
    "qt_argsort_desc": (c_int, [c_void_p, c_int, c_void_p, c_void_p, c_void_p]),
    "qt_cholesky_inverse_upper_workspace_bytes": (c_size_t, [c_int]),
    "qt_cholesky_inverse_upper": (c_int, [c_void_p, c_int, c_void_p, c_void_p, c_void_p, c_size_t, c_void_p]),
    "qt_cholesky_inverse_upper_batched_workspace_bytes": (c_size_t, [c_int, c_int]),
    "qt_cholesky_inverse_upper_batched": (c_int, [c_void_p, c_int64, c_int, c_void_p, c_int64, c_void_p, c_int, c_void_p,
                                                  c_size_t, c_void_p]),
    "qt_cholesky_inverse_upper_bounded": (c_int, [c_void_p, c_int, c_void_p, c_void_p, c_void_p, c_void_p, c_size_t,
                                                  c_void_p]),
    "qt_cholesky_inverse_upper_batched_bounded": (c_int, [c_void_p, c_int64, c_int, c_void_p, c_int64, c_void_p, c_int,
                                                          c_void_p, c_void_p, c_size_t, c_void_p]),
    "qt_group_minmax_qparams": (c_int, [c_void_p, c_int, c_int, c_int, c_int64, c_int, c_int, c_int, c_void_p,
                                        c_void_p, c_void_p, c_void_p, c_void_p]),
    "qt_weight_gather_f32": (c_int, [c_void_p, c_int, c_int, c_int, c_int64, c_void_p, c_void_p, c_void_p,
                                     c_void_p]),
    "qt_weight_gather_qparams": (c_int, [c_void_p, c_int, c_int, c_int, c_int64, c_void_p, c_void_p, c_int, c_int, c_int,
                                         c_void_p, c_void_p, c_void_p, c_void_p, c_void_p, c_int64, c_void_p]),
    "qt_gptq_sweep_workspace_bytes": (c_size_t, [c_int, c_int, c_int]),
    "qt_gptq_sweep": (c_int, [c_void_p, c_int, c_int, c_void_p, c_void_p, c_void_p, c_int, c_void_p, c_int, c_int,
                              c_void_p, c_void_p, c_void_p, c_size_t, c_void_p]),
    "qt_gptq_sweep_grouped": (c_int, [c_void_p, c_int, c_int, c_void_p, c_int64, c_int, c_void_p, c_void_p, c_void_p, c_int,
                                      c_void_p, c_int, c_int, c_void_p, c_void_p, c_void_p, c_size_t, c_void_p]),
    "qt_pack_int4": (c_int, [c_void_p, c_int, c_int, c_void_p, c_void_p, c_void_p]),
    "qt_awq_weight_mean_workspace_bytes": (c_size_t, [c_int, c_int]),
    "qt_awq_weight_mean_accumulate": (c_int, [c_void_p, c_int, c_int, c_int, c_int64, c_int, c_void_p, c_void_p,
                                              c_size_t, c_void_p]),
    "qt_awq_scales": (c_int, [c_void_p, c_int64, c_void_p, c_int64, c_int, c_int, c_int, c_void_p, c_void_p]),
    "qt_symmetrize_lower": (c_int, [c_void_p, c_int, c_void_p]),
    "qt_awq_loss_workspace_bytes": (c_size_t, [c_int, c_int]),
    "qt_awq_loss": (c_int, [c_void_p, c_int, c_int, c_int, c_int64, c_void_p, c_int, c_int, c_int, c_void_p, c_int64,
                            c_int, c_float, c_int, c_void_p, c_void_p, c_size_t, c_void_p]),
    "qt_awq_losses_workspace_bytes": (c_size_t, [c_int, c_int, c_int]),
    "qt_awq_losses": (c_int, [c_void_p, c_int, c_int, c_int, c_int64, c_void_p, c_int, c_int, c_int, c_int, c_void_p,
                              c_int64, c_float, c_int, c_void_p, c_void_p, c_size_t, c_void_p]),
    "qt_argmin_f32": (c_int, [c_void_p, c_int, c_void_p, c_void_p]),
    "qt_awq_pseudo_quantize": (c_int, [c_void_p, c_int, c_int, c_int, c_int64, c_void_p, c_int, c_int, c_int, c_void_p,
                                       c_int64, c_void_p]),
    "qt_scale_columns": (c_int, [c_void_p, c_int, c_int, c_int, c_int64, c_void_p, c_int, c_void_p, c_int64,
                                 c_void_p]),
    "qt_rtn_quantize": (c_int, [c_void_p, c_int, c_int, c_int, c_int64, c_void_p, c_void_p, c_int, c_int, c_int,
                                c_void_p, c_void_p]),
    "qt_col_absmax_workspace_bytes": (c_size_t, [c_int, c_int]),
    "qt_col_absmax_accumulate": (c_int, [c_void_p, c_int, c_int, c_int, c_int64, c_void_p, c_void_p, c_size_t,
                                         c_void_p]),
    "qt_smoothquant_scales": (c_int, [c_void_p, c_void_p, c_void_p, c_int, c_float, c_void_p, c_void_p]),
    "qt_xtx_dot_workspace_bytes": (c_size_t, [c_int64, c_int]),
    "qt_xtx_dot": (c_int, [c_void_p, c_int, c_int64, c_int, c_int64, c_void_p, c_double, c_void_p, c_int, c_void_p,
                           c_size_t, c_void_p]),
    "qt_gemm3_plan_check": (c_int, [c_int, c_int, c_int, c_int, c_void_p, c_void_p, c_void_p]),
    "qt_xtx_tile_table_check": (c_int, [c_int, c_void_p, c_void_p, c_void_p]),
    "qt_chol_g3_plan_check": (c_int, [c_int, c_int, c_int, c_void_p]),
    "qt_gemm3_tn_f32_workspace_bytes": (c_size_t, [c_int, c_int, c_int]),
    "qt_gemm3_tn_f32": (c_int, [c_void_p, c_int64, c_void_p, c_int64, c_void_p, c_int64, c_int, c_int, c_int, c_int,
                                c_void_p, c_size_t, c_void_p]),
    "qt_gemm3_tn_f32_ex": (c_int, [c_void_p, c_int64, c_void_p, c_int64, c_void_p, c_int64, c_int, c_int, c_int, c_int,
                                   c_int, c_int, c_int, c_int64, c_int64, c_int64, c_void_p, c_size_t, c_void_p]),
    "qt_gemm3_tn_f16x2": (c_int, [c_void_p, c_int64, c_void_p, c_int64, c_void_p, c_int64, c_int, c_int, c_int, c_int,
                                  c_int, c_int, c_int, c_int64, c_int64, c_int64, c_void_p, c_void_p, c_void_p, c_size_t,
                                  c_void_p]),
    "qt_sgemm_tn_f32_workspace_bytes": (c_size_t, [c_int, c_int]),
    "qt_sgemm_tn_f32": (c_int, [c_void_p, c_int64, c_void_p, c_int64, c_void_p, c_int64, c_void_p, c_int64, c_int,
                                c_int, c_int, c_int, c_int, c_int, c_void_p, c_size_t, c_void_p]),
    "qt_profile_enable": (c_int, [c_int]),
    "qt_profile_read": (c_int, [c_int, c_void_p, c_void_p]),
    "qt_dequantize": (c_int, [c_void_p, c_int, c_int, c_void_p, c_void_p, c_void_p, c_int, c_void_p, c_void_p,
                              c_int, c_int64, c_void_p]),
    "qt_quantize_tokens_i8": (c_int, [c_void_p, c_int, c_int64, c_int, c_int64, c_void_p, c_int, c_void_p, c_void_p,
                                      c_void_p, c_void_p]),
    "qt_act_mul_quantize_i8": (c_int, [c_void_p, c_int64, c_void_p, c_int64, c_int, c_int64, c_int, c_int, c_void_p,
                                       c_int, c_void_p, c_void_p, c_void_p, c_void_p, c_int64, c_void_p]),
    "qt_rmsnorm_quantize_i8": (c_int, [c_void_p, c_int64, c_void_p, c_int, c_int64, c_int, c_float, c_void_p, c_int,
                                       c_void_p, c_void_p, c_void_p, c_void_p, c_int64, c_void_p, c_void_p]),
    "qt_gemm_i8": (c_int, [c_void_p, c_int64, c_int, c_void_p, c_int, c_int, c_void_p, c_void_p, c_void_p, c_int,
                           c_void_p, c_void_p, c_void_p, c_int, c_int64, c_void_p]),
    "qt_gemm_i8_skinny": (c_int, [c_void_p, c_int, c_int, c_void_p, c_int, c_int, c_void_p, c_void_p, c_void_p, c_int,
                                  c_void_p, c_void_p, c_void_p, c_int, c_int64, c_void_p]),
    "qt_gemm_i8_ring": (c_int, [c_void_p, c_int64, c_int, c_void_p, c_int, c_int, c_void_p, c_void_p, c_void_p, c_int,
                                c_void_p, c_void_p, c_void_p, c_int, c_int64, c_void_p]),
    "qt_gemm_i8_ring_w4": (c_int, [c_void_p, c_int64, c_int, c_void_p, c_int, c_int, c_void_p, c_void_p, c_void_p,
                                   c_int, c_void_p, c_void_p, c_void_p, c_int, c_int64, c_void_p]),
    "qt_gemm_i8_mid": (c_int, [c_void_p, c_int64, c_int, c_void_p, c_int, c_int, c_void_p, c_void_p, c_void_p, c_int,
                               c_void_p, c_void_p, c_void_p, c_int, c_int64, c_void_p]),
    "qt_splitk_gemm_i8_plan": (c_int, [c_int64, c_int, c_int, c_int, c_int, c_void_p, c_void_p]),
    "qt_splitk_gemm_i8_range": (c_int, [c_int, c_int, c_int, c_void_p, c_void_p]),
    "qt_splitk_gemm_i8": (c_int, [c_void_p, c_int64, c_int, c_void_p, c_int, c_int, c_void_p, c_void_p, c_void_p, c_int,
                                  c_void_p, c_void_p, c_void_p, c_int, c_int64, c_int, c_void_p, c_size_t, c_void_p]),
    "qt_gemm_i8_skinny_grouped": (c_int, [c_void_p, c_int, c_void_p, c_int64, c_void_p, c_int, c_void_p, c_int, c_int,
                                          c_void_p, c_void_p, c_void_p, c_int, c_void_p, c_void_p, c_int, c_int64,
                                          c_void_p]),
    "qt_moe_route": (c_int, [c_void_p, c_int, c_int64, c_int, c_int, c_void_p, c_void_p, c_void_p, c_void_p,
                             c_void_p]),
    "qt_gemm_i8_grouped": (c_int, [c_void_p, c_int, c_void_p, c_int64, c_void_p, c_int, c_void_p, c_int, c_int,
                                   c_void_p, c_void_p, c_void_p, c_int, c_void_p, c_void_p, c_int, c_int64, c_void_p]),
    "qt_gemm_i8_ring_grouped": (c_int, [c_void_p, c_int, c_void_p, c_int64, c_void_p, c_int, c_void_p, c_int, c_int,
                                        c_void_p, c_void_p, c_void_p, c_int, c_void_p, c_void_p, c_int, c_int64,
                                        c_int64, c_void_p]),
    "qt_moe_gemm_i8_ring_w4": (c_int, [c_void_p, c_int, c_void_p, c_int64, c_void_p, c_int, c_void_p, c_int, c_int,
                                       c_void_p, c_void_p, c_void_p, c_int, c_void_p, c_void_p, c_int, c_int64,
                                       c_int64, c_void_p]),
    "qt_moe_gemm_i8_wide": (c_int, [c_void_p, c_int, c_void_p, c_int64, c_void_p, c_int, c_void_p, c_int, c_int,
                                    c_void_p, c_void_p, c_void_p, c_int, c_void_p, c_void_p, c_int, c_int64,
                                    c_int64, c_void_p]),
    "qt_moe_combine": (c_int, [c_void_p, c_int, c_int, c_int64, c_void_p, c_void_p, c_int64, c_int, c_void_p,
                               c_void_p]),
    "qt_dequantize_weight": (c_int, [c_void_p, c_int, c_int, c_int, c_void_p, c_int, c_void_p, c_void_p, c_void_p,
                                     c_int, c_int64, c_void_p]),
    "qt_gemm_wq_skinny": (c_int, [c_void_p, c_int, c_int, c_int, c_int64, c_void_p, c_int, c_int, c_void_p, c_int,
                                  c_void_p, c_void_p, c_void_p, c_void_p, c_int64, c_void_p]),
    "qt_gemm_wq_stream": (c_int, [c_void_p, c_int, c_int, c_int, c_int64, c_void_p, c_int, c_int, c_void_p, c_int,
                                  c_void_p, c_void_p, c_void_p, c_void_p, c_int64, c_void_p]),
    "qt_gemm_wq_grouped": (c_int, [c_void_p, c_int, c_int, c_int64, c_void_p, c_int64, c_void_p, c_int, c_void_p,
                                   c_int, c_int, c_void_p, c_int, c_void_p, c_void_p, c_void_p, c_int64, c_void_p]),
    "qt_moe_gemm_wq_wide": (c_int, [c_void_p, c_int, c_int, c_int64, c_void_p, c_int64, c_void_p, c_int, c_void_p,
                                    c_int, c_int, c_void_p, c_int, c_void_p, c_void_p, c_void_p, c_int64, c_int64,
                                    c_void_p]),
    "qt_lm_head_nll_workspace_size": (c_size_t, [c_int64, c_int]),
    "qt_lm_head_nll": (c_int, [c_void_p, c_int64, c_void_p, c_int64, c_int, c_int64, c_int, c_int, c_void_p, c_int,
                               c_void_p, c_void_p, c_void_p, c_void_p, c_void_p, c_size_t, c_void_p]),
    "qt_lm_head_kl_workspace_size": (c_size_t, [c_int64, c_int]),
    "qt_lm_head_kl": (c_int, [c_void_p, c_int64, c_void_p, c_int64, c_void_p, c_int64, c_int, c_int64, c_int, c_int,
                              c_void_p, c_int, c_void_p, c_void_p, c_void_p, c_void_p, c_void_p, c_void_p, c_void_p,
                              c_void_p, c_size_t, c_void_p]),
}

_lib = None


class HipBackendError(RuntimeError):

    def __init__(self, fn: str, status: int, message: str):
        super().__init__(f"{fn} failed with status {status}: {message}")
        self.status = status


# ... 26 lines not shown
```

### quantool_amd/hip/ops.py

```python
from __future__ import annotations

import ctypes
import logging
import os
from collections import namedtuple
from dataclasses import dataclass
from typing import Optional

import torch

from . import _lib
from ._lib import QT_BF16, QT_F16, QT_F32, HipBackendError, check, load

_WS_CACHE: dict = {}


def _stream() -> int:
    return torch.cuda.current_stream().cuda_stream


def _ptr(t: Optional[torch.Tensor]) -> Optional[int]:
    return None if t is None else t.data_ptr()


def _dtype_code(t: torch.Tensor) -> int:
    if t.dtype == torch.float32:
        return QT_F32
    if t.dtype == torch.bfloat16:
        return QT_BF16
    if t.dtype == torch.float16:
        return QT_F16
    raise TypeError(f"unsupported dtype {t.dtype} (fp32 / bf16 / fp16 only)")


def _act16(X: torch.Tensor, name: str) -> int:
    if not X.is_cuda:
        raise ValueError(f"{name} must be a device tensor (no CPU path exists)")
    if X.dtype not in (torch.bfloat16, torch.float16):
        raise TypeError(f"{name} must be bf16 or fp16, got {X.dtype}")
    return QT_BF16 if X.dtype == torch.bfloat16 else QT_F16


def _rows16(X2: torch.Tensor) -> torch.Tensor:
    if X2.stride(1) != 1 or X2.data_ptr() % 16 or (X2.shape[0] > 1 and X2.stride(0) % 8):
        X2 = X2.contiguous()
    return X2


_FP32_ACT_WARNED = False


def as_act16(X: torch.Tensor) -> torch.Tensor:
    if X.dtype in (torch.bfloat16, torch.float16):
        return X
    wide_activation_policy(X.dtype)
    return X.to(torch.bfloat16)


def wide_gram_mode() -> str:
    mode = os.environ.get("QT_FP32_ACTIVATIONS", "exact").lower()
    if mode not in ("exact", "bf16", "warn", "error"):
        raise ValueError(f"QT_FP32_ACTIVATIONS={mode!r}: expected exact, bf16 or error")
    return "bf16" if mode == "warn" else mode


def wide_activation_policy(dtype) -> None:
    if dtype not in (torch.float32, torch.float64):
        raise TypeError(f"calibration activations must be floating point, got {dtype}")
    global _FP32_ACT_WARNED
    policy = os.environ.get("QT_FP32_ACTIVATIONS", "exact").lower()
    if policy == "error":
        raise ValueError(f"{dtype} calibration activations: this backend accumulates X^T X from 16-bit activations; "
                         "load the model in bf16 / fp16 (oneshot(precision=...)) or unset QT_FP32_ACTIVATIONS=error to "
                         "accept rounding them to bf16")
    if not _FP32_ACT_WARNED:
        _FP32_ACT_WARNED = True
        logging.getLogger(__name__).warning(
            f"{dtype} calibration activations are rounded to bf16 for the Gram / statistics passes (upstream accumulates "
            "them in fp32): Hessians differ at the 2^-9 level per activation.  Load the model in bf16 / fp16 to calibrate "
            "in its own dtype, or set QT_FP32_ACTIVATIONS=error to refuse")


def _req(t: torch.Tensor, dtype, name: str, ndim: Optional[int] = None):
    if not t.is_cuda:
        raise ValueError(f"{name} must be a device tensor (no CPU path exists)")
    if t.dtype != dtype:
        raise TypeError(f"{name} must be {dtype}, got {t.dtype}")
    if ndim is not None and t.dim() != ndim:
        raise ValueError(f"{name} must be {ndim}-d, got shape {tuple(t.shape)}")


def workspace(nbytes: int, device, tag: str = "default") -> torch.Tensor:
    key = (str(device), _stream(), tag)
    buf = _WS_CACHE.get(key)
    if buf is None or buf.numel() < nbytes:
        buf = torch.empty(max(nbytes, 1), dtype=torch.uint8, device=device)
        _WS_CACHE[key] = buf
    return buf


def release_workspaces() -> None:
    _WS_CACHE.clear()


def xtx_accumulate(X: torch.Tensor, G: torch.Tensor) -> None:
    lib = load()
    xdt = _act16(X, "X")
    _req(G, torch.float32, "G", 2)
    K = G.shape[0]
    if G.shape[1] != K or not G.is_contiguous():
        raise ValueError("G must be contiguous [K, K]")
    if X.shape[-1] != K:
        raise ValueError(f"X last dim {X.shape[-1]} != K {K}")
    X2 = _rows16(X.reshape(-1, K))
    n = X2.shape[0]
    if n == 0:
        return
    ldx = X2.stride(0) if n > 1 else K
    nbytes = lib.qt_xtx_workspace_bytes(n, K)
    ws = workspace(nbytes, X.device, "xtx")
    check("qt_xtx_accumulate", lib.qt_xtx_accumulate(X2.data_ptr(), xdt, n, K, ldx, G.data_ptr(), ws.data_ptr(),
                                                     ws.numel(), _stream()))


XTX_BATCH_MAX = 16


def xtx_batched_plan(n_tokens, K: int):
    import ctypes

    lib = load()
    n = len(n_tokens)
    counts = (ctypes.c_int64 * n)(*[int(t) for t in n_tokens])
    n_items, n_slabs = ctypes.c_int(0), ctypes.c_int(0)
    check("qt_xtx_batched_plan", lib.qt_xtx_batched_plan(counts, n, K, None, 0, ctypes.byref(n_items),
                                                         ctypes.byref(n_slabs), None))
    rows = (ctypes.c_int32 * (6 * max(1, n_items.value)))()
    check("qt_xtx_batched_plan", lib.qt_xtx_batched_plan(counts, n, K, rows, n_items.value, ctypes.byref(n_items),
                                                         ctypes.byref(n_slabs), None))
    return [tuple(rows[6 * i:6 * i + 6]) for i in range(n_items.value)], n_slabs.value


def xtx_batched_workspace_bytes(n_tokens, K: int) -> int:
    import ctypes

    n = len(n_tokens)
    counts = (ctypes.c_int64 * n)(*[int(t) for t in n_tokens])
    need = ctypes.c_size_t(0)
    check("qt_xtx_batched_plan", load().qt_xtx_batched_plan(counts, n, K, None, 0, None, None, ctypes.byref(need)))
    return int(need.value)


def xtx_accumulate_batched(Xs, Gs) -> None:
    import ctypes

    lib = load()
    Xs, Gs = list(Xs), list(Gs)
    if len(Xs) != len(Gs):
        raise ValueError(f"{len(Xs)} inputs for {len(Gs)} Gram matrices")
    if not Xs:
        return
    xdt = _act16(Xs[0], "Xs[0]")
    K = Gs[0].shape[0]
    batch = []
    for i, (X, G) in enumerate(zip(Xs, Gs)):
        if _act16(X, f"Xs[{i}]") != xdt:
            raise TypeError(f"Xs[{i}] is {X.dtype}, Xs[0] is {Xs[0].dtype}: one dtype per batch")
        _req(G, torch.float32, f"Gs[{i}]", 2)
        if tuple(G.shape) != (K, K) or not G.is_contiguous():
            raise ValueError(f"Gs[{i}] must be contiguous [{K}, {K}], got {tuple(G.shape)}")
        if X.shape[-1] != K:
            raise ValueError(f"Xs[{i}] last dim {X.shape[-1]} != K {K}")
        if X.device != Xs[0].device or G.device != Xs[0].device:
            raise ValueError(f"problem {i} is not on {Xs[0].device}: one device per batch")
        if any(G.data_ptr() == g.data_ptr() for _, g in batch):
            raise ValueError(f"Gs[{i}] is also an earlier problem's Gram matrix")
        X2 = _rows16(X.reshape(-1, K))
        n = X2.shape[0]
        if n == 0:
            continue
        if n % 64 and n > 1 and X2.stride(0) != K:
            xtx_accumulate(X2, G)
            continue
        batch.append((X2, G))
    for b0 in range(0, len(batch), XTX_BATCH_MAX):
        part = batch[b0:b0 + XTX_BATCH_MAX]
        m = len(part)
        counts = (ctypes.c_int64 * m)(*[x.shape[0] for x, _ in part])
        pitches = (ctypes.c_int64 * m)(*[x.stride(0) if x.shape[0] > 1 else K for x, _ in part])
        xp = (ctypes.c_void_p * m)(*[x.data_ptr() for x, _ in part])
        gp = (ctypes.c_void_p * m)(*[g.data_ptr() for _, g in part])
        ws = workspace(xtx_batched_workspace_bytes([x.shape[0] for x, _ in part], K), Xs[0].device, "xtx_batched")
        check("qt_xtx_accumulate_batched", lib.qt_xtx_accumulate_batched(xp, xdt, counts, pitches, K, gp, m, ws.data_ptr(),
                                                                         ws.numel(), _stream()))


def xtx_accumulate_f32(X: torch.Tensor, G: torch.Tensor) -> None:
    lib = load()
    _req(X, torch.float32, "X")
    _req(G, torch.float32, "G", 2)
    K = G.shape[0]
    if G.shape[1] != K or not G.is_contiguous():
        raise ValueError("G must be contiguous [K, K]")
    if X.shape[-1] != K:
        raise ValueError(f"X last dim {X.shape[-1]} != K {K}")
# ... 72 lines not shown
        if perm.numel() != K or not perm.is_contiguous():
            raise ValueError("perm must be contiguous int32[K]")
    A = A_out if A_out is not None else torch.empty((K, K), dtype=torch.float32, device=G.device)
    _req(A, torch.float32, "A", 2)
    if A.shape != (K, K) or not A.is_contiguous():
        raise ValueError("A must be contiguous [K, K]")
    dead = torch.empty(K, dtype=torch.uint8, device=G.device)
    diag = torch.empty(K, dtype=torch.float32, device=G.device)
    need = lib.qt_hessian_prepare_workspace_bytes(K)
    if scratch is not None and scratch.is_cuda and scratch.is_contiguous() and scratch.numel() * scratch.element_size() >= need:
        ws = scratch.view(torch.uint8).reshape(-1)
    else:
        ws = workspace(need, G.device, "prep")
    if damp_out is not None:
        _req(damp_out, torch.float32, "damp_out", damp_out.dim())
        if damp_out.numel() < 1 or damp_out.device != G.device:
            raise ValueError("damp_out must be a non-empty fp32 tensor on G's device")
        check("qt_hessian_prepare_damp", lib.qt_hessian_prepare_damp(
            G.data_ptr(), K, int(n_samples), float(percdamp), _ptr(perm), A.data_ptr(), dead.data_ptr(), diag.data_ptr(),
            damp_out.data_ptr(), ws.data_ptr(), ws.numel(), _stream()))
        return A, dead, diag
    check("qt_hessian_prepare", lib.qt_hessian_prepare(G.data_ptr(), K, int(n_samples), float(percdamp), _ptr(perm),
                                                       A.data_ptr(), dead.data_ptr(), diag.data_ptr(), ws.data_ptr(),
                                                       ws.numel(), _stream()))
    return A, dead, diag


def _min_eig_lb(lb: torch.Tensor, n: int, device) -> torch.Tensor:
    _req(lb, torch.float32, "min_eig_lb", lb.dim())
    if lb.numel() != n or not lb.is_contiguous() or lb.device != device:
        raise ValueError(f"min_eig_lb must be a contiguous fp32 device tensor of {n} value(s)")
    return lb


def cholesky_inverse_upper(A: torch.Tensor, U_out: Optional[torch.Tensor] = None,
                           min_eig_lb: Optional[torch.Tensor] = None):
    lib = load()
    _req(A, torch.float32, "A", 2)
    K = A.shape[0]
    if A.shape != (K, K) or not A.is_contiguous():
        raise ValueError("A must be contiguous [K, K]")
    U = U_out if U_out is not None else torch.empty((K, K), dtype=torch.float32, device=A.device)
    if U.shape != (K, K) or not U.is_contiguous() or U.dtype != torch.float32:
        raise ValueError("U must be contiguous fp32 [K, K]")
    info = torch.zeros(1, dtype=torch.int32, device=A.device)
    ws = workspace(lib.qt_cholesky_inverse_upper_workspace_bytes(K), A.device, "chol")
    if min_eig_lb is not None:
        lb = _min_eig_lb(min_eig_lb, 1, A.device)
        check("qt_cholesky_inverse_upper_bounded", lib.qt_cholesky_inverse_upper_bounded(
            A.data_ptr(), K, U.data_ptr(), info.data_ptr(), lb.data_ptr(), ws.data_ptr(), ws.numel(), _stream()))
        return U, info
    check("qt_cholesky_inverse_upper", lib.qt_cholesky_inverse_upper(A.data_ptr(), K, U.data_ptr(), info.data_ptr(),
                                                                     ws.data_ptr(), ws.numel(), _stream()))
    return U, info


MAX_BATCH = 16


def cholesky_inverse_upper_batched(A: torch.Tensor, U: torch.Tensor, min_eig_lb: Optional[torch.Tensor] = None):
    lib = load()
    _req(A, torch.float32, "A", 3)
    _req(U, torch.float32, "U", 3)
    n, K, K2 = A.shape
    if K != K2 or tuple(U.shape) != (n, K, K) or not (1 <= n <= MAX_BATCH):
        raise ValueError(f"A / U must be [n <= {MAX_BATCH}, K, K], got {tuple(A.shape)} / {tuple(U.shape)}")
    for name, t in (("A", A), ("U", U)):
        if t.stride(2) != 1 or t.stride(1) != K or (n > 1 and (t.stride(0) < K * K or t.stride(0) % 4)):
            raise ValueError(f"{name}: every [b] slice must be a contiguous K x K matrix at a stride that is a multiple of 4")
    info = torch.zeros(n, dtype=torch.int32, device=A.device)
    ws = workspace(lib.qt_cholesky_inverse_upper_batched_workspace_bytes(K, n), A.device, "chol")
    if min_eig_lb is not None:
        lb = _min_eig_lb(min_eig_lb, n, A.device)
        check("qt_cholesky_inverse_upper_batched_bounded", lib.qt_cholesky_inverse_upper_batched_bounded(
            A.data_ptr(), A.stride(0) if n > 1 else K * K, K, U.data_ptr(), U.stride(0) if n > 1 else K * K,
            info.data_ptr(), n, lb.data_ptr(), ws.data_ptr(), ws.numel(), _stream()))
        return info
    check("qt_cholesky_inverse_upper_batched", lib.qt_cholesky_inverse_upper_batched(
        A.data_ptr(), A.stride(0) if n > 1 else K * K, K, U.data_ptr(), U.stride(0) if n > 1 else K * K, info.data_ptr(), n,
        ws.data_ptr(), ws.numel(), _stream()))
    return info


def group_minmax_qparams(W: torch.Tensor, group_size: int, symmetric: bool = True, num_bits: int = 4):
    lib = load()
    if W.dim() != 2 or not W.is_cuda or W.stride(1) != 1:
        raise ValueError("W must be a 2-d device tensor with unit column stride")
    R, K = W.shape
    gs = K if group_size <= 0 else group_size
    if K % gs:
        raise ValueError(f"K={K} not divisible by group_size={gs}")
    G = K // gs
    dev = W.device
    scale = torch.empty((R, G), dtype=torch.float32, device=dev)
    zp = torch.empty((R, G), dtype=torch.float32, device=dev)
    scale_t = torch.empty((G, R), dtype=torch.float32, device=dev)
    zp_t = torch.empty((G, R), dtype=torch.float32, device=dev)
    check("qt_group_minmax_qparams", lib.qt_group_minmax_qparams(
        W.data_ptr(), _dtype_code(W), R, K, W.stride(0), gs, int(bool(symmetric)), num_bits, scale.data_ptr(),
        zp.data_ptr(), scale_t.data_ptr(), zp_t.data_ptr(), _stream()))
    return scale, zp, scale_t, zp_t


def weight_gather_f32(W: torch.Tensor, perm: Optional[torch.Tensor] = None, dead: Optional[torch.Tensor] = None,
                      out: Optional[torch.Tensor] = None) -> torch.Tensor:
    lib = load()
    if W.dim() != 2 or not W.is_cuda or W.stride(1) != 1:
        raise ValueError("W must be a 2-d device tensor with unit column stride")
    R, K = W.shape
    if perm is not None:
        _req(perm, torch.int32, "perm", 1)
        assert perm.numel() == K and perm.is_contiguous()
    if dead is not None:
        _req(dead, torch.uint8, "dead", 1)
        assert dead.numel() == K and dead.is_contiguous()
    if out is None:
        out = torch.empty((R, K), dtype=torch.float32, device=W.device)
    assert out.shape == (R, K) and out.is_contiguous() and out.dtype == torch.float32
    check("qt_weight_gather_f32", lib.qt_weight_gather_f32(W.data_ptr(), _dtype_code(W), R, K, W.stride(0),
                                                           _ptr(perm), _ptr(dead), out.data_ptr(), _stream()))
    return out


def weight_gather_qparams(W: torch.Tensor, perm: Optional[torch.Tensor], dead: Optional[torch.Tensor], group_size: int,
                          symmetric: bool, num_bits: int, out: torch.Tensor, scale: torch.Tensor, zp: torch.Tensor,
                          scale_t: Optional[torch.Tensor] = None, zp_t: Optional[torch.Tensor] = None) -> None:
    lib = load()
    if W.dim() != 2 or not W.is_cuda or W.stride(1) != 1:
        raise ValueError("W must be a 2-d device tensor with unit column stride")
    R, K = W.shape
    gs = K if group_size <= 0 else group_size
    if K % gs:
        raise ValueError(f"K={K} not divisible by group_size={gs}")
    G = K // gs
    for name, t, shape in (("out", out, (R, K)), ("scale", scale, (R, G)), ("zp", zp, (R, G))):
        _req(t, torch.float32, name, 2)
        if tuple(t.shape) != shape or not t.is_contiguous():
            raise ValueError(f"{name} must be contiguous {shape}")
    ld_t = 0
    for name, t in (("scale_t", scale_t), ("zp_t", zp_t)):
        if t is not None:
            _req(t, torch.float32, name, 2)
            if tuple(t.shape) != (G, R) or t.stride(1) != 1 or (ld_t and t.stride(0) != ld_t):
                raise ValueError(f"{name} must be a [G, R] view with unit column stride (and the row stride of its twin)")
            ld_t = t.stride(0) if G > 1 else max(R, t.stride(0))
    for name, t, dt in (("perm", perm, torch.int32), ("dead", dead, torch.uint8)):
        if t is not None:
            _req(t, dt, name, 1)
            if t.numel() != K or not t.is_contiguous():
                raise ValueError(f"{name} must be contiguous [K]")
    check("qt_weight_gather_qparams", lib.qt_weight_gather_qparams(
        W.data_ptr(), _dtype_code(W), R, K, W.stride(0), _ptr(perm), _ptr(dead), group_size, int(bool(symmetric)), num_bits,
        out.data_ptr(), scale.data_ptr(), zp.data_ptr(), _ptr(scale_t), _ptr(zp_t), ld_t, _stream()))


def gptq_sweep(W: torch.Tensor, U: torch.Tensor, scale_t: torch.Tensor, zp_t: torch.Tensor, g_idx: torch.Tensor,
               blocksize: int = 128, num_bits: int = 4):
    lib = load()
    _req(W, torch.float32, "W", 2)
    _req(U, torch.float32, "U", 2)
    _req(scale_t, torch.float32, "scale_t", 2)
    _req(zp_t, torch.float32, "zp_t", 2)
    _req(g_idx, torch.int32, "g_idx", 1)
    R, K = W.shape
    G = scale_t.shape[0]
    if not (W.is_contiguous() and U.is_contiguous() and scale_t.is_contiguous() and zp_t.is_contiguous()
            and g_idx.is_contiguous()):
        raise ValueError("all sweep operands must be contiguous")
    if U.shape != (K, K) or scale_t.shape != (G, R) or zp_t.shape != (G, R) or g_idx.numel() != K:
        raise ValueError("sweep operand shapes inconsistent")
    Qt = torch.empty((K, R), dtype=torch.int8, device=W.device)
    loss = torch.empty(R, dtype=torch.float32, device=W.device)
    ws = workspace(lib.qt_gptq_sweep_workspace_bytes(R, K, blocksize), W.device, "sweep")
    check("qt_gptq_sweep", lib.qt_gptq_sweep(W.data_ptr(), R, K, U.data_ptr(), scale_t.data_ptr(), zp_t.data_ptr(), G,
                                             g_idx.data_ptr(), blocksize, num_bits, Qt.data_ptr(), loss.data_ptr(),
                                             ws.data_ptr(), ws.numel(), _stream()))
    return Qt, loss


def gptq_sweep_grouped(W: torch.Tensor, U: torch.Tensor, row_end, scale_t: torch.Tensor, zp_t: torch.Tensor,
                       g_idx: torch.Tensor, blocksize: int = 128, num_bits: int = 4):
    import ctypes

    lib = load()
    _req(W, torch.float32, "W", 2)
    _req(U, torch.float32, "U", 3)
    _req(scale_t, torch.float32, "scale_t", 2)
    _req(zp_t, torch.float32, "zp_t", 2)
    _req(g_idx, torch.int32, "g_idx", 2)
    R, K = W.shape
    n = U.shape[0]
    G = scale_t.shape[0]
    row_end = [int(r) for r in row_end]
    if not (W.is_contiguous() and scale_t.is_contiguous() and zp_t.is_contiguous() and g_idx.is_contiguous()):
        raise ValueError("all sweep operands must be contiguous")
    if (tuple(U.shape) != (n, K, K) or U.stride(2) != 1 or U.stride(1) != K or scale_t.shape != (G, R) or zp_t.shape != (G, R)
            or tuple(g_idx.shape) != (n, K) or len(row_end) != n or not (1 <= n <= MAX_BATCH)):
        raise ValueError("grouped sweep operand shapes inconsistent")
    if row_end[-1] != R or any(b <= a for a, b in zip([0] + row_end[:-1], row_end)) or any(r % 128 for r in row_end[:-1]):
        raise ValueError(f"row_end={row_end}: ascending, every boundary but the last a multiple of 128, last == R ({R})")
    Qt = torch.empty((K, R), dtype=torch.int8, device=W.device)
    loss = torch.empty(R, dtype=torch.float32, device=W.device)
    ws = workspace(lib.qt_gptq_sweep_workspace_bytes(R, K, blocksize), W.device, "sweep")
    ends = (ctypes.c_int32 * n)(*row_end)
    check("qt_gptq_sweep_grouped", lib.qt_gptq_sweep_grouped(
        W.data_ptr(), R, K, U.data_ptr(), U.stride(0) if n > 1 else K * K, n, ctypes.cast(ends, ctypes.c_void_p),
        scale_t.data_ptr(), zp_t.data_ptr(), G, g_idx.data_ptr(), blocksize, num_bits, Qt.data_ptr(), loss.data_ptr(),
        ws.data_ptr(), ws.numel(), _stream()))
    return Qt, loss


def pack_int4(Qt: torch.Tensor, col_src: Optional[torch.Tensor] = None) -> torch.Tensor:
    lib = load()
    _req(Qt, torch.int8, "Qt", 2)
    K, R = Qt.shape
    assert Qt.is_contiguous()
    if col_src is not None:
        _req(col_src, torch.int32, "col_src", 1)
        assert col_src.numel() == K and col_src.is_contiguous()
    packed = torch.empty((R, (K + 7) // 8), dtype=torch.int32, device=Qt.device)
    check("qt_pack_int4", lib.qt_pack_int4(Qt.data_ptr(), R, K, _ptr(col_src), packed.data_ptr(), _stream()))
    return packed


def dequantize(Qt: torch.Tensor, scale: torch.Tensor, zp: torch.Tensor, g_of_col: torch.Tensor,
               col_src: Optional[torch.Tensor] = None, dtype=torch.float32) -> torch.Tensor:
    lib = load()
    _req(Qt, torch.int8, "Qt", 2)
    K, R = Qt.shape
    _req(scale, torch.float32, "scale", 2)
    _req(zp, torch.float32, "zp", 2)
    _req(g_of_col, torch.int32, "g_of_col", 1)
    G = scale.shape[1]
    assert scale.shape == (R, G) and zp.shape == (R, G) and g_of_col.numel() == K
    assert Qt.is_contiguous() and scale.is_contiguous() and zp.is_contiguous() and g_of_col.is_contiguous()
    if col_src is not None:
        _req(col_src, torch.int32, "col_src", 1)
        assert col_src.numel() == K and col_src.is_contiguous()
    out = torch.empty((R, K), dtype=dtype, device=Qt.device)
    check("qt_dequantize", lib.qt_dequantize(Qt.data_ptr(), R, K, _ptr(col_src), scale.data_ptr(), zp.data_ptr(), G,
                                             g_of_col.data_ptr(), out.data_ptr(), _dtype_code(out), out.stride(0),
                                             _stream()))
    return out


def _x2d(X: torch.Tensor, name: str) -> int:
    code = _act16(X, name)
    if X.dim() != 2 or X.stride(1) != 1:
        raise ValueError(f"{name} must be 2-d [rows, columns] with unit column stride, got shape {tuple(X.shape)} "
                         f"strides {X.stride()}")
    return code


def quantize_tokens_i8(X: torch.Tensor, symmetric: bool = True, col_perm: Optional[torch.Tensor] = None):
    lib = load()
    code = _x2d(X, "X")
    M, K = X.shape
    if M == 0 or K == 0:
        raise ValueError(f"X must be non-empty, got shape {tuple(X.shape)}")
    if col_perm is not None:
        _req(col_perm, torch.int32, "col_perm", 1)
        if col_perm.numel() != K or not col_perm.is_contiguous():
            raise ValueError(f"col_perm must be contiguous int32 [{K}]")
    Xq = torch.empty((M, K), dtype=torch.int8, device=X.device)
    s_x = torch.empty(M, dtype=torch.float32, device=X.device)
    zp_x = None if symmetric else torch.empty(M, dtype=torch.int32, device=X.device)
    check("qt_quantize_tokens_i8", lib.qt_quantize_tokens_i8(
        X.data_ptr(), code, M, K, X.stride(0), _ptr(col_perm), int(bool(symmetric)), Xq.data_ptr(), s_x.data_ptr(),
        _ptr(zp_x), _stream()))
    return Xq, s_x, zp_x


ACTS = {"silu": 0}


def act_mul_quantize_i8(gate: torch.Tensor, up: torch.Tensor, symmetric: bool = True,
                        col_perm: Optional[torch.Tensor] = None, act: str = "silu", return_h: bool = False):
    lib = load()
    code = _x2d(gate, "gate")
    if _x2d(up, "up") != code or up.shape != gate.shape or up.device != gate.device:
        raise ValueError(f"gate and up must agree in shape, dtype and device, got {tuple(gate.shape)} {gate.dtype} "
                         f"and {tuple(up.shape)} {up.dtype}")
    if act not in ACTS:
        raise ValueError(f"act must be one of {sorted(ACTS)}, got {act!r}")
    M, K = gate.shape
    if M == 0 or K == 0:
        raise ValueError(f"gate must be non-empty, got shape {tuple(gate.shape)}")
    if col_perm is not None:
        _req(col_perm, torch.int32, "col_perm", 1)
        if col_perm.numel() != K or not col_perm.is_contiguous():
            raise ValueError(f"col_perm must be contiguous int32 [{K}]")
    Xq = torch.empty((M, K), dtype=torch.int8, device=gate.device)
    s_x = torch.empty(M, dtype=torch.float32, device=gate.device)
    zp_x = None if symmetric else torch.empty(M, dtype=torch.int32, device=gate.device)
    H = torch.empty((M, K), dtype=gate.dtype, device=gate.device) if return_h else None
    ldg = gate.stride(0) if M > 1 else max(gate.stride(0), K)
    ldu = up.stride(0) if M > 1 else max(up.stride(0), K)
    check("qt_act_mul_quantize_i8", lib.qt_act_mul_quantize_i8(
        gate.data_ptr(), ldg, up.data_ptr(), ldu, code, M, K, ACTS[act], _ptr(col_perm), int(bool(symmetric)),
        Xq.data_ptr(), s_x.data_ptr(), _ptr(zp_x), _ptr(H), K, _stream()))
    return (Xq, s_x, zp_x, H) if return_h else (Xq, s_x, zp_x)


def rmsnorm_quantize_i8(X: torch.Tensor, weight: torch.Tensor, eps: float, symmetric: bool = True,
                        col_perm: Optional[torch.Tensor] = None, return_rstd: bool = False):
# ... 1009 lines not shown
```

Baseline: 3.271 billion.

## Add xtx set mode, stacked int4 pack with scale cast, row-wise flat reverse

Adds a set variant of the X^T X kernel that writes G directly and zeroes the mirrored tile, so the caller no longer has to zero and then accumulate. Adds a stacked int4 pack kernel that packs every segment of the stacked Qt in one launch and also writes the dtype-converted scales, replacing per-weight contiguous slices, pack launches and casts. The lower-to-upper flat reverse in Cholesky is rewritten to one block per row pair with vectorized f32x4 swaps. These are several unrelated launch-count and memory-traffic reductions, and they add new env toggles and more code paths to keep correct.

```diff
diff --git a/include/quantool_amd.h b/include/quantool_amd.h
--- a/include/quantool_amd.h
+++ b/include/quantool_amd.h
@@ -27,6 +27,8 @@
 size_t qt_xtx_workspace_bytes(int64_t n_tokens, int K);
 int qt_xtx_accumulate(const void* X, int x_dtype, int64_t n_tokens, int K, int64_t ldx, float* G,
                       void* workspace, size_t workspace_bytes, qt_stream_t stream);
+int qt_xtx_set(const void* X, int x_dtype, int64_t n_tokens, int K, int64_t ldx, float* G, void* workspace,
+               size_t workspace_bytes, qt_stream_t stream);
 
 int qt_xtx_accumulate_batched(const void* const* X, int x_dtype, const int64_t* n_tokens, const int64_t* ldx, int K,
                               float* const* G, int n_problems, void* workspace, size_t workspace_bytes,
@@ -90,6 +92,10 @@
 
 int qt_pack_int4(const int8_t* Qt, int R, int K, const int32_t* col_src, int32_t* packed,
                  qt_stream_t stream);
+int qt_pack_int4_stacked(const int8_t* Qt, int R_total, int K, const float* scale, int G, int n_segments,
+                         const int32_t* seg_row0, const int32_t* seg_rows, const int32_t* const* seg_col_src,
+                         int32_t* const* seg_packed, void* const* seg_scale_out, const int32_t* seg_scale_dtype,
+                         qt_stream_t stream);
 
 int qt_dequantize(const int8_t* Qt, int R, int K, const int32_t* col_src, const float* scale,
                   const float* zp, int G, const int32_t* g_of_col, void* out, int out_dtype,
@@ -149,6 +155,7 @@
 
 int qt_gemm3_plan_check(int Tm, int Tn, int c_end, int tri, int* n_items_out, int* n_slabs_out, int* longest_out);
 int qt_chol_g3_plan_check(int K, int merged, int min_chunks, long long* counts_out);
+int qt_chol_flat_reverse(float* Y, int K, int n_problems, int64_t stride, qt_stream_t stream);
 enum qt_act { QT_ACT_SILU = 0 };
 #define QT_I8_MID_MAX_M 128
 #define QT_I8_MID_K_UNIT 128
diff --git a/quantool_amd/csrc/cholesky.hip b/quantool_amd/csrc/cholesky.hip
--- a/quantool_amd/csrc/cholesky.hip
+++ b/quantool_amd/csrc/cholesky.hip
@@ -554,23 +554,45 @@
     }
 }
 
+template <bool VEC>
 __global__ __launch_bounds__(256) void flat_reverse_lower_to_upper_kernel(float* __restrict__ U, int K, int64_t bsU) {
     U += (size_t)blockIdx.z * bsU;
-    const int j = blockIdx.x * blockDim.x + threadIdx.x;
-    const int i = blockIdx.y;
-    if (j >= K || j < i) return;
-    const size_t e = (size_t)i * K + j;
-    const size_t pe = (size_t)(K - 1 - i) * K + (K - 1 - j);
-    if (i == j) {
-        if (e <= pe) {
-            const float t = U[e];
-            U[e] = U[pe];
-            U[pe] = t;
+    const int i = blockIdx.x, ip = K - 1 - i;
+    float* ri = U + (size_t)i * K;
+    float* rp = U + (size_t)ip * K;
+    if constexpr (VEC) {
+        for (int j = 4 * (int)threadIdx.x; j < K; j += 4 * 256) {
+            const int m = K - 4 - j;
+            f32x4 a = {0.f, 0.f, 0.f, 0.f}, b = {0.f, 0.f, 0.f, 0.f};
+            if (j <= i) a = *(const f32x4*)(ri + j);
+            if (m <= ip) b = *(const f32x4*)(rp + m);
+            f32x4 oi, op;
+#pragma unroll
+            for (int e = 0; e < 4; ++e) {
+                oi[e] = (j + e >= i) ? b[3 - e] : 0.0f;
+                op[e] = (m + e >= ip) ? a[3 - e] : 0.0f;
+            }
+            *(f32x4*)(ri + j) = oi;
+            *(f32x4*)(rp + m) = op;
         }
     } else {
-        U[e] = U[pe];
-        U[pe] = 0.0f;
-    }
+        const int jend = (i == ip) ? (K + 1) / 2 : K;
+        for (int j = threadIdx.x; j < jend; j += 256) {
+            const int m = K - 1 - j;
+            const float a = ri[j], b = rp[m];
+            ri[j] = (j >= i) ? b : 0.0f;
+            rp[m] = (m >= ip) ? a : 0.0f;
+        }
+    }
+}
+
+static int chol_flat_reverse(float* U, int K, int nprob, int64_t bsU, hipStream_t stream) {
+    if (K % 4 == 0 && ((uintptr_t)U & 15) == 0 && bsU % 4 == 0)
+        hipLaunchKernelGGL(flat_reverse_lower_to_upper_kernel<true>, dim3(K / 2, 1, nprob), dim3(256), 0, stream, U, K, bsU);
+    else
+        hipLaunchKernelGGL(flat_reverse_lower_to_upper_kernel<false>, dim3((K + 1) / 2, 1, nprob), dim3(256), 0, stream, U, K, bsU);
+    QT_LAUNCH_CHECK();
+    return QT_OK;
 }
 
 __global__ __launch_bounds__(256) void identity_if_failed_kernel(float* __restrict__ U, int K,
@@ -903,8 +925,7 @@
         QT_LAUNCH_CHECK();
     }
     if (int rc = c.merge_mode == CHOL_TWO_PHASE ? chol_run_two_phase(c) : chol_run_walk(c)) return rc;
-    hipLaunchKernelGGL(flat_reverse_lower_to_upper_kernel, dim3((K + 255) / 256, K, nprob), dim3(256), 0, stream, U, K, c.sY);
-    QT_LAUNCH_CHECK();
+    if (int rc = chol_flat_reverse(U, K, nprob, c.sY, stream)) return rc;
     hipLaunchKernelGGL(identity_if_failed_kernel, dim3(K < 1024 ? K : 1024, 1, nprob), dim3(256), 0, stream, U, K,
                        (const int32_t*)info, c.sY);
     QT_LAUNCH_CHECK();
@@ -917,6 +938,12 @@
     QT_CHECK_ARG(n_problems == 1 || (strideA >= (int64_t)K * K && strideU >= (int64_t)K * K && strideA % 4 == 0 && strideU % 4 == 0),
                  "%s: strides must be multiples of 4 elements and >= K*K", fn);
     return QT_OK;
+}
+
+extern "C" int qt_chol_flat_reverse(float* Y, int K, int n_problems, int64_t stride, qt_stream_t stream_) {
+    QT_CHECK_ARG(Y && K > 0 && n_problems >= 1 && (n_problems == 1 || stride >= (int64_t)K * K),
+                 "qt_chol_flat_reverse: bad arguments");
+    return chol_flat_reverse(Y, K, n_problems, n_problems > 1 ? stride : 0, (hipStream_t)stream_);
 }
 
 extern "C" int qt_cholesky_inverse_upper(float* A, int K, float* U, int32_t* info, void* workspace,
diff --git a/quantool_amd/csrc/quant.hip b/quantool_amd/csrc/quant.hip
--- a/quantool_amd/csrc/quant.hip
+++ b/quantool_amd/csrc/quant.hip
@@ -1,3 +1,5 @@
+#include <string.h>
+
 #include "common.h"
 
 namespace {
@@ -205,6 +207,89 @@
         const int wl = e & 31, rl = e >> 5;
         const int r = r0 + rl, w = w0 + wl;
         if (r < R && w < Kw) packed[(size_t)r * Kw + w] = (int32_t)tile[rl][wl];
+    }
+}
+
+constexpr int PACK_MAX_SEGS = 48;
+struct PackSegs {
+    int n;
+    int tile0[PACK_MAX_SEGS + 1];
+    int row0[PACK_MAX_SEGS], rows[PACK_MAX_SEGS], rows4[PACK_MAX_SEGS], scale_dtype[PACK_MAX_SEGS];
+    const int32_t* col_src[PACK_MAX_SEGS];
+    int32_t* packed[PACK_MAX_SEGS];
+    void* scale_out[PACK_MAX_SEGS];
+};
+
+__global__ __launch_bounds__(256) void pack_int4_stacked_kernel(const int8_t* __restrict__ Qt, int Rt, int K,
+                                                                const float* __restrict__ scale, int G, PackSegs sg) {
+    __shared__ uint32_t tile[256][33];
+    int s = 0;
+    while (s + 1 < sg.n && (int)blockIdx.y >= sg.tile0[s + 1]) ++s;
+    const int row0 = sg.row0[s], rows = sg.rows[s];
+    const bool four = sg.rows4[s] != 0;
+    const int th = four ? 256 : 64;
+    const int rl0 = ((int)blockIdx.y - sg.tile0[s]) * th;
+    const int32_t* __restrict__ col_src = sg.col_src[s];
+    int32_t* __restrict__ packed = sg.packed[s];
+    const int Kw = (K + 7) / 8;
+    const int w0 = blockIdx.x * 32;
+    const int tid = threadIdx.x;
+    const int8_t* __restrict__ q0 = Qt + row0;
+    if (four) {
+        for (int e = tid; e < 64 * 32; e += 256) {
+            const int rq = e & 63, wl = e >> 6;
+            const int r = rl0 + 4 * rq, w = w0 + wl;
+            uint32_t acc[4] = {0, 0, 0, 0};
+            if (r < rows && w < Kw) {
+#pragma unroll
+                for (int j = 0; j < 8; ++j) {
+                    const int c = w * 8 + j;
+                    if (c < K) {
+                        const int sc = col_src ? col_src[c] : c;
+                        const uint32_t q4 = *(const uint32_t*)(q0 + (size_t)sc * Rt + r);
+#pragma unroll
+                        for (int i = 0; i < 4; ++i) {
+                            const uint32_t u = (uint32_t)((int)(int8_t)(q4 >> (8 * i)) + 8) & 0xFu;
+                            acc[i] |= u << (4 * j);
+                        }
+                    }
+                }
+            }
+#pragma unroll
+            for (int i = 0; i < 4; ++i) tile[4 * rq + i][wl] = acc[i];
+        }
+    } else {
+        for (int e = tid; e < 64 * 32; e += 256) {
+            const int rl = e & 63, wl = e >> 6;
+            const int r = rl0 + rl, w = w0 + wl;
+            uint32_t acc = 0;
+            if (r < rows && w < Kw) {
+#pragma unroll
+                for (int j = 0; j < 8; ++j) {
+                    const int c = w * 8 + j;
+                    if (c < K) {
+                        const int sc = col_src ? col_src[c] : c;
+                        const uint32_t u = ((uint32_t)((int)q0[(size_t)sc * Rt + r] + 8)) & 0xFu;
+                        acc |= u << (4 * j);
+                    }
+                }
+            }
+            tile[rl][wl] = acc;
+        }
+    }
+    __syncthreads();
+    for (int e = tid; e < th * 32; e += 256) {
+        const int wl = e & 31, rl = e >> 5;
+        const int r = rl0 + rl, w = w0 + wl;
+        if (r < rows && w < Kw) packed[(size_t)r * Kw + w] = (int32_t)tile[rl][wl];
+    }
+    void* so = sg.scale_out[s];
+    if (so) {
+        const int dt = sg.scale_dtype[s];
+        const int nr = rows - rl0 < th ? rows - rl0 : th;
+        const size_t n = (size_t)nr * G, d0 = (size_t)rl0 * G;
+        const float* __restrict__ src = scale + (size_t)(row0 + rl0) * G;
+        for (size_t e = (size_t)blockIdx.x * 256 + tid; e < n; e += (size_t)gridDim.x * 256) qt_store_w(so, dt, d0 + e, src[e]);
     }
 }
 
@@ -339,6 +424,49 @@
     return QT_OK;
 }
 
+extern "C" int qt_pack_int4_stacked(const int8_t* Qt, int R_total, int K, const float* scale, int G, int n_segments,
+                                    const int32_t* seg_row0, const int32_t* seg_rows, const int32_t* const* seg_col_src,
+                                    int32_t* const* seg_packed, void* const* seg_scale_out, const int32_t* seg_scale_dtype,
+                                    qt_stream_t stream_) {
+    hipStream_t stream = (hipStream_t)stream_;
+    QT_CHECK_ARG(Qt && R_total > 0 && K > 0 && n_segments > 0 && seg_row0 && seg_rows && seg_packed,
+                 "qt_pack_int4_stacked: bad arguments");
+    const int Kw = (K + 7) / 8;
+    const bool stack4 = R_total % 4 == 0 && (((uintptr_t)Qt) & 3) == 0;
+    for (int s = 0; s < n_segments; ++s) {
+        QT_CHECK_ARG(seg_rows[s] > 0 && seg_row0[s] >= 0 && (int64_t)seg_row0[s] + seg_rows[s] <= R_total && seg_packed[s],
+                     "qt_pack_int4_stacked: segment %d (rows [%d, +%d)) does not lie inside the %d stacked rows", s, seg_row0[s],
+                     seg_rows[s], R_total);
+        if (seg_scale_out && seg_scale_out[s])
+            QT_CHECK_ARG(scale && G > 0 && seg_scale_dtype && qt_dtype_ok(seg_scale_dtype[s]),
+                         "qt_pack_int4_stacked: segment %d has a scale tensor but no scale table / dtype", s);
+    }
+    for (int s0 = 0; s0 < n_segments; s0 += PACK_MAX_SEGS) {
+        PackSegs sg;
+        memset(&sg, 0, sizeof(sg));
+        sg.n = n_segments - s0 < PACK_MAX_SEGS ? n_segments - s0 : PACK_MAX_SEGS;
+        int tiles = 0;
+        for (int i = 0; i < sg.n; ++i) {
+            const int s = s0 + i;
+            sg.tile0[i] = tiles;
+            sg.row0[i] = seg_row0[s];
+            sg.rows[i] = seg_rows[s];
+            sg.rows4[i] = stack4 && seg_row0[s] % 4 == 0;
+            tiles += (seg_rows[s] + (sg.rows4[i] ? 255 : 63)) / (sg.rows4[i] ? 256 : 64);
+            sg.col_src[i] = seg_col_src ? seg_col_src[s] : nullptr;
+            sg.packed[i] = seg_packed[s];
+            sg.scale_out[i] = seg_scale_out ? seg_scale_out[s] : nullptr;
+            sg.scale_dtype[i] = sg.scale_out[i] ? seg_scale_dtype[s] : QT_F32;
+        }
+        sg.tile0[sg.n] = tiles;
+        QT_CHECK_ARG(tiles <= 65535, "qt_pack_int4_stacked: %d row tiles in one launch (at most 65535)", tiles);
+        hipLaunchKernelGGL(pack_int4_stacked_kernel, dim3((Kw + 31) / 32, tiles), dim3(256), 0, stream, Qt, R_total, K, scale, G,
+                           sg);
+        QT_LAUNCH_CHECK();
+    }
+    return QT_OK;
+}
+
 extern "C" int qt_dequantize(const int8_t* Qt, int R, int K, const int32_t* col_src, const float* scale,
                              const float* zp, int G, const int32_t* g_of_col, void* out, int out_dtype, int64_t ldo,
                              qt_stream_t stream_) {
diff --git a/quantool_amd/csrc/xtx.hip b/quantool_amd/csrc/xtx.hip
--- a/quantool_amd/csrc/xtx.hip
+++ b/quantool_amd/csrc/xtx.hip
@@ -39,7 +39,16 @@
     int64_t x_batch_bytes;
     const struct XtxBItem* b_items;
     const struct XtxBProb* b_probs;
+    int set;
 };
+
+__device__ __forceinline__ void xtx_zero_mirror_tile(float* G, int K, int ti, int tj, int tid) {
+    const f32x4 z = {0.f, 0.f, 0.f, 0.f};
+    for (int e = tid; e < BT * (BT / 4); e += NTHREADS) {
+        const int gi = tj * BT + e / (BT / 4), gj = ti * BT + (e % (BT / 4)) * 4;
+        if (gi < K && gj < K) *(f32x4*)(G + (size_t)gi * K + gj) = z;
+    }
+}
 
 struct XtxBItem {
     int prob;
@@ -279,7 +288,20 @@
     }
 
     const int jl = lane & 31, ih = 4 * (lane >> 5);
-    if (slab_idx < 0) {
+    if (slab_idx < 0 && p.set) {
+#pragma unroll
+        for (int mi = 0; mi < 4; ++mi)
+#pragma unroll
+            for (int ni = 0; ni < 2; ++ni) {
+                const int gj = tj * BT + wave_n * 64 + ni * 32 + jl;
+#pragma unroll
+                for (int r = 0; r < 16; ++r) {
+                    const int gi = ti * BT + wave_m * 128 + mi * 32 + (r & 3) + 8 * (r >> 2) + ih;
+                    if (gi < K && gj < K) p.G[(size_t)gi * K + gj] = acc[mi][ni][r];
+                }
+            }
+        if (ti != tj) xtx_zero_mirror_tile(p.G, K, ti, tj, tid);
+    } else if (slab_idx < 0) {
 #pragma unroll
         for (int mi = 0; mi < 4; ++mi)
 #pragma unroll
@@ -482,7 +504,20 @@
         }
         return;
     }
-    if (slab_idx < 0) {
+    if (slab_idx < 0 && p.set) {
+#pragma unroll
+        for (int ai = 0; ai < 8; ++ai)
+#pragma unroll
+            for (int bj = 0; bj < 4; ++bj) {
+                const int gj = tj * BT + wave_n * 64 + bj * 16 + jl;
+#pragma unroll
+                for (int r = 0; r < 4; ++r) {
+                    const int gi = ti * BT + wave_m * 128 + ai * 16 + ih + r;
+                    if (gi < K && gj < K) Gp[(size_t)gi * K + gj] = acc[ai][bj][r];
+                }
+            }
+        if (ti != tj) xtx_zero_mirror_tile(Gp, K, ti, tj, tid);
+    } else if (slab_idx < 0) {
 #pragma unroll
         for (int ai = 0; ai < 8; ++ai)
 #pragma unroll
@@ -514,7 +549,7 @@
 
 __global__ __launch_bounds__(256) void xtx_reduce_kernel(const float* __restrict__ slabs, int n_rem, int n_splits,
                                                          float* __restrict__ G, int K,
-                                                         const int* __restrict__ tile_tab) {
+                                                         const int* __restrict__ tile_tab, int set) {
     const int tile = blockIdx.x;
     const int tt_packed = tile_tab[tile];
     const int ti = tt_packed >> 16, tj = tt_packed & 0xFFFF;
@@ -524,6 +559,10 @@
         const int i_loc = part * 16 + e / (BT / 4);
         const int j_loc = (e % (BT / 4)) * 4;
         const int gi = ti * BT + i_loc, gj = tj * BT + j_loc;
+        if (set && ti != tj) {
+            const int mi = tj * BT + i_loc, mj = ti * BT + j_loc;
+            if (mi < K && mj + 3 < K) *(f32x4*)(G + (size_t)mi * K + mj) = f32x4{0.f, 0.f, 0.f, 0.f};
+        }
         if (gi >= K || gj >= K) continue;
         f32x4 s = {0.f, 0.f, 0.f, 0.f};
         for (int sp = 0; sp < n_splits; ++sp) {
@@ -532,7 +571,11 @@
             s += v;
         }
         float* dst = G + (size_t)gi * K + gj;
-        if (gj + 3 < K) {
+        if (set) {
+            if (gj + 3 < K) *(f32x4*)dst = s;
+            else
+                for (int c = 0; c < 4 && gj + c < K; ++c) dst[c] = s[c];
+        } else if (gj + 3 < K) {
             f32x4 o = *(f32x4*)dst;
             o += s;
             *(f32x4*)dst = o;
@@ -730,14 +773,19 @@
     return pl.slab_bytes + pl.tail_bytes + pl.tab_bytes + pl.prog_bytes + 256;
 }
 
-extern "C" int qt_xtx_accumulate(const void* X, int x_dtype, int64_t n_tokens, int K, int64_t ldx, float* G,
-                                 void* workspace, size_t workspace_bytes, qt_stream_t stream_) {
-    hipStream_t stream = (hipStream_t)stream_;
+static int xtx_run(const void* X, int x_dtype, int64_t n_tokens, int K, int64_t ldx, float* G, void* workspace,
+                   size_t workspace_bytes, hipStream_t stream, int set) {
     QT_CHECK_ARG(qt_dtype_is16(x_dtype), "qt_xtx_accumulate: x_dtype %d must be QT_BF16 or QT_F16", x_dtype);
     QT_CHECK_ARG(K > 0 && K % 8 == 0, "qt_xtx_accumulate: K=%d must be a positive multiple of 8", K);
     QT_CHECK_ARG(ldx >= K && ldx % 8 == 0, "qt_xtx_accumulate: ldx=%lld must be >= K and a multiple of 8", (long long)ldx);
     QT_CHECK_ARG(n_tokens >= 0, "qt_xtx_accumulate: n_tokens < 0");
-    if (n_tokens == 0) return QT_OK;
+    if (n_tokens == 0) {
+        if (set) {
+            QT_CHECK_ARG(G, "qt_xtx_set: null pointer");
+            QT_HIP(hipMemsetAsync(G, 0, (size_t)K * K * sizeof(float), stream));
+        }
+        return QT_OK;
+    }
     QT_CHECK_ARG(X && G, "qt_xtx_accumulate: null pointer");
     QT_CHECK_ARG(((uintptr_t)X & 15) == 0 && ((uintptr_t)G & 15) == 0, "qt_xtx_accumulate: X and G must be 16-byte aligned");
     QT_CHECK_ARG((uint64_t)ldx * 2 * UT + (uint64_t)K * 2 < ((uint64_t)1 << 32), "qt_xtx_accumulate: ldx too large");
@@ -782,6 +830,9 @@
     p.dot_partials = nullptr;
     p.batch_items = 1;
     p.x_batch_bytes = 0;
+    p.b_items = nullptr;
+    p.b_probs = nullptr;
+    p.set = set;
     p.wrap_units = 0;
 #ifdef QT_XTX_ABLATION
     {
@@ -839,7 +890,7 @@
         QT_LAUNCH_CHECK();
         if (ql.n_rem > 0) {
             hipLaunchKernelGGL(xtx_reduce_kernel, dim3(ql.n_rem, 16), dim3(256), 0, stream, q.slabs, ql.n_rem, ql.s2,
-                               q.G, q.K, q.tile_tab + ql.n_direct);
+                               q.G, q.K, q.tile_tab + ql.n_direct, q.set);
             QT_LAUNCH_CHECK();
         }
         return QT_OK;
@@ -875,9 +926,20 @@
         ptp.n_direct = pt.n_direct;
         ptp.n_rem = 0;
         ptp.s2 = 1;
+        ptp.set = set && full == 0;
         return launch(ptp, pt);
     }
     return launch(p, pl);
+}
+
+extern "C" int qt_xtx_accumulate(const void* X, int x_dtype, int64_t n_tokens, int K, int64_t ldx, float* G,
+                                 void* workspace, size_t workspace_bytes, qt_stream_t stream_) {
+    return xtx_run(X, x_dtype, n_tokens, K, ldx, G, workspace, workspace_bytes, (hipStream_t)stream_, 0);
+}
+
+extern "C" int qt_xtx_set(const void* X, int x_dtype, int64_t n_tokens, int K, int64_t ldx, float* G, void* workspace,
+                          size_t workspace_bytes, qt_stream_t stream_) {
+    return xtx_run(X, x_dtype, n_tokens, K, ldx, G, workspace, workspace_bytes, (hipStream_t)stream_, 1);
 }
 
 namespace {
@@ -1258,6 +1320,9 @@
     p.dot_partials = partials;
     p.batch_items = items;
     p.x_batch_bytes = x_batch_stride * 2;
+    p.b_items = nullptr;
+    p.b_probs = nullptr;
+    p.set = 0;
     const int grid = items * n_batch;
     qt_prof_mark(QT_PROF_XTX, stream);
     if (x_dtype == QT_F16) hipLaunchKernelGGL((xtx16_kernel<true, true>), dim3(grid), dim3(NTHREADS), 0, stream, p);
diff --git a/quantool_amd/engine/gptq_linear.py b/quantool_amd/engine/gptq_linear.py
--- a/quantool_amd/engine/gptq_linear.py
+++ b/quantool_amd/engine/gptq_linear.py
@@ -17,7 +17,10 @@
     def __init__(self, K: int, device, stage_tokens: Optional[int] = None, dtype: Optional[torch.dtype] = None):
         self.K = K
         self.dtype = dtype
-        self._G = torch.zeros((K, K), dtype=torch.float32, device=device)
+        self._G = torch.empty((K, K), dtype=torch.float32, device=device)
+        self._fresh = True
+        if not ops.xtx_set_enabled(self._G):
+            self._zero_if_fresh()
         self.n = 0
         if stage_tokens is None:
             stage_tokens = max(4096, min(65536, self.STAGE_BYTES // (2 * K)))
@@ -32,7 +35,13 @@
     def G(self) -> torch.Tensor:
         self.flush()
         self._after_flush()
+        self._zero_if_fresh()
         return self._G
+
+    def _zero_if_fresh(self) -> None:
+        if self._fresh:
+            self._G.zero_()
+            self._fresh = False
 
     def _after_flush(self) -> None:
         if self._flushed is not None:
@@ -44,6 +53,7 @@
     @G.setter
     def G(self, value: torch.Tensor) -> None:
         self._G = value
+        self._fresh = False
 
     def add(self, X: torch.Tensor, num_samples: Optional[int] = None) -> None:
         if num_samples is None:
@@ -87,6 +97,11 @@
         else:
             chunks = [rows[t0:t0 + limit] for t0 in range(0, rows.shape[0], limit)]
         for part in chunks:
+            if part.dtype != torch.float32 and self._fresh and ops.xtx_set_enabled(self._G):
+                ops.xtx_set(part, self._G)
+                self._fresh = False
+                continue
+            self._zero_if_fresh()
             if part.dtype == torch.float32:
                 ops.xtx_accumulate_f32(part, self._G)
             else:
@@ -129,6 +144,7 @@
                     if here is not None and acc._staged_on is not None and here != acc._staged_on:
                         here.wait_stream(acc._staged_on)
                     acc._after_flush()
+                    acc._zero_if_fresh()
                 ops.xtx_accumulate_batched([acc._stage[:acc._fill] for acc in run], [acc._G for acc in run])
                 event = here.record_event() if here is not None else None
                 for acc in run:
@@ -145,7 +161,11 @@
         self._after_flush()
         self._fill = 0
         self._staged_on = self._flushed = None
-        self._G.zero_()
+        if ops.xtx_set_enabled(self._G):
+            self._fresh = True
+        else:
+            self._fresh = False
+            self._G.zero_()
         self.n = 0
 
 
@@ -193,8 +213,8 @@
             raise RuntimeError("the integer levels of this result were released (sequential driver, "
                                "QT_RESULT_DETAIL_BYTES): the module's weight holds the dequantised values")
         if self.Qt.device.type == "cpu":
-            return ops.dequantize(*_on_device(self.Qt, self.scale_f32, self.zp_f32, self.g_of_col, self.col_src), dtype).cpu()
-        return ops.dequantize(self.Qt, self.scale_f32, self.zp_f32, self.g_of_col, self.col_src, dtype)
+            return ops.dequantize(*_on_device(self.Qt.contiguous(), self.scale_f32, self.zp_f32, self.g_of_col, self.col_src), dtype).cpu()
+        return ops.dequantize(self.Qt.contiguous(), self.scale_f32, self.zp_f32, self.g_of_col, self.col_src, dtype)
 
 
 def _normalize_actorder(actorder) -> Optional[str]:
@@ -341,6 +361,20 @@
                                           qargs.num_bits)
     del Wf, U, ubuf
 
+    def scale_dtype_of(w):
+        return scale_dtype or (w.dtype if w.dtype in (torch.bfloat16, torch.float16) else torch.float32)
+
+    stacked = None
+    if qargs.num_bits == 4 and ops.pack_stacked_enabled():
+        segs = []
+        for b, (ws, acc) in enumerate(groups):
+            r0 = row_begin[b]
+            for w, r in zip(ws, rows[b]):
+                sdt = scale_dtype_of(w)
+                segs.append((r0, r, invs[b], None if sdt == torch.float32 else sdt))
+                r0 += r
+        stacked = iter(ops.pack_int4_stacked(Qt, segs, scale.contiguous()))
+
     results: List[List[GPTQResult]] = []
     for b, (ws, acc) in enumerate(groups):
         col_src = invs[b]
@@ -351,16 +385,23 @@
         out: List[GPTQResult] = []
         r0 = row_begin[b]
         for w, r in zip(ws, rows[b]):
-            Qt_i = Qt[:, r0:r0 + r].contiguous() if R > r else Qt
-            sdt = scale_dtype or (w.dtype if w.dtype in (torch.bfloat16, torch.float16) else torch.float32)
+            sdt = scale_dtype_of(w)
             sc_i = scale[r0:r0 + r].contiguous()
             zp_i = zp[r0:r0 + r].contiguous()
-            packed = ops.pack_int4(Qt_i, col_src) if qargs.num_bits == 4 else None
+            if stacked is not None:
+                Qt_i = Qt[:, r0:r0 + r]
+                packed, w_scale = next(stacked)
+                if w_scale is None:
+                    w_scale = sc_i
+            else:
+                Qt_i = Qt[:, r0:r0 + r].contiguous() if R > r else Qt
+                packed = ops.pack_int4(Qt_i, col_src) if qargs.num_bits == 4 else None
+                w_scale = sc_i.to(sdt)
             wq = None
             if packed is None:
                 wq = (Qt_i.t() if col_src is None else Qt_i[col_src.long()].t()).contiguous()
             out.append(GPTQResult(
-                weight_packed=packed, weight_q=wq, weight_scale=sc_i.to(sdt),
+                weight_packed=packed, weight_q=wq, weight_scale=w_scale,
                 weight_zero_point=None if qargs.symmetric else zp_i.to(torch.int8),
                 weight_g_idx=g_of_col if actorder == "group" else None,
                 weight_shape=torch.tensor([r, K], dtype=torch.int64), loss=loss[r0:r0 + r], info=info[b:b + 1],
diff --git a/quantool_amd/hip/_lib.py b/quantool_amd/hip/_lib.py
--- a/quantool_amd/hip/_lib.py
+++ b/quantool_amd/hip/_lib.py
@@ -22,6 +22,7 @@
     "qt_last_error": (c_char_p, []),
     "qt_xtx_workspace_bytes": (c_size_t, [c_int64, c_int]),
     "qt_xtx_accumulate": (c_int, [c_void_p, c_int, c_int64, c_int, c_int64, c_void_p, c_void_p, c_size_t, c_void_p]),
+    "qt_xtx_set": (c_int, [c_void_p, c_int, c_int64, c_int, c_int64, c_void_p, c_void_p, c_size_t, c_void_p]),
     "qt_xtx_accumulate_batched": (c_int, [c_void_p, c_int, c_void_p, c_void_p, c_int, c_void_p, c_int, c_void_p, c_size_t,
                                           c_void_p]),
     "qt_xtx_batched_plan": (c_int, [c_void_p, c_int, c_int, c_void_p, c_int, c_void_p, c_void_p, c_void_p]),
@@ -58,6 +59,8 @@
     "qt_gptq_sweep_grouped": (c_int, [c_void_p, c_int, c_int, c_void_p, c_int64, c_int, c_void_p, c_void_p, c_void_p, c_int,
                                       c_void_p, c_int, c_int, c_void_p, c_void_p, c_void_p, c_size_t, c_void_p]),
     "qt_pack_int4": (c_int, [c_void_p, c_int, c_int, c_void_p, c_void_p, c_void_p]),
+    "qt_pack_int4_stacked": (c_int, [c_void_p, c_int, c_int, c_void_p, c_int, c_int, c_void_p, c_void_p, c_void_p, c_void_p,
+                                     c_void_p, c_void_p, c_void_p]),
     "qt_awq_weight_mean_workspace_bytes": (c_size_t, [c_int, c_int]),
     "qt_awq_weight_mean_accumulate": (c_int, [c_void_p, c_int, c_int, c_int, c_int64, c_int, c_void_p, c_void_p,
                                               c_size_t, c_void_p]),
@@ -86,6 +89,7 @@
     "qt_gemm3_plan_check": (c_int, [c_int, c_int, c_int, c_int, c_void_p, c_void_p, c_void_p]),
     "qt_xtx_tile_table_check": (c_int, [c_int, c_void_p, c_void_p, c_void_p]),
     "qt_chol_g3_plan_check": (c_int, [c_int, c_int, c_int, c_void_p]),
+    "qt_chol_flat_reverse": (c_int, [c_void_p, c_int, c_int, c_int64, c_void_p]),
     "qt_gemm3_tn_f32_workspace_bytes": (c_size_t, [c_int, c_int, c_int]),
     "qt_gemm3_tn_f32": (c_int, [c_void_p, c_int64, c_void_p, c_int64, c_void_p, c_int64, c_int, c_int, c_int, c_int,
                                 c_void_p, c_size_t, c_void_p]),
diff --git a/quantool_amd/hip/ops.py b/quantool_amd/hip/ops.py
--- a/quantool_amd/hip/ops.py
+++ b/quantool_amd/hip/ops.py
@@ -104,6 +104,20 @@
 
 
 def xtx_accumulate(X: torch.Tensor, G: torch.Tensor) -> None:
+    _xtx("qt_xtx_accumulate", X, G)
+
+
+def xtx_set(X: torch.Tensor, G: torch.Tensor) -> None:
+    _xtx("qt_xtx_set", X, G)
+
+
+def xtx_set_enabled(G: torch.Tensor) -> bool:
+    import os
+
+    return G.is_cuda and os.environ.get("QT_XTX_SET", "1") != "0"
+
+
+def _xtx(fn: str, X: torch.Tensor, G: torch.Tensor) -> None:
     lib = load()
     xdt = _act16(X, "X")
     _req(G, torch.float32, "G", 2)
@@ -115,12 +129,13 @@
     X2 = _rows16(X.reshape(-1, K))
     n = X2.shape[0]
     if n == 0:
+        if fn == "qt_xtx_set":
+            G.zero_()
         return
     ldx = X2.stride(0) if n > 1 else K
     nbytes = lib.qt_xtx_workspace_bytes(n, K)
     ws = workspace(nbytes, X.device, "xtx")
-    check("qt_xtx_accumulate", lib.qt_xtx_accumulate(X2.data_ptr(), xdt, n, K, ldx, G.data_ptr(), ws.data_ptr(),
-                                                     ws.numel(), _stream()))
+    check(fn, getattr(lib, fn)(X2.data_ptr(), xdt, n, K, ldx, G.data_ptr(), ws.data_ptr(), ws.numel(), _stream()))
 
 
 XTX_BATCH_MAX = 16
@@ -359,6 +374,17 @@
     return info
 
 
+def chol_flat_reverse(Y: torch.Tensor) -> torch.Tensor:
+    lib = load()
+    _req(Y, torch.float32, "Y")
+    Y3 = Y if Y.dim() == 3 else Y.unsqueeze(0)
+    n, K, K2 = Y3.shape
+    if K != K2 or Y3.stride(2) != 1 or Y3.stride(1) != K or (n > 1 and Y3.stride(0) < K * K):
+        raise ValueError("Y: contiguous K x K matrices at a uniform stride >= K * K")
+    check("qt_chol_flat_reverse", lib.qt_chol_flat_reverse(Y3.data_ptr(), K, n, Y3.stride(0) if n > 1 else K * K, _stream()))
+    return Y
+
+
 def group_minmax_qparams(W: torch.Tensor, group_size: int, symmetric: bool = True, num_bits: int = 4):
     lib = load()
     if W.dim() != 2 or not W.is_cuda or W.stride(1) != 1:
@@ -498,6 +524,53 @@
     packed = torch.empty((R, (K + 7) // 8), dtype=torch.int32, device=Qt.device)
     check("qt_pack_int4", lib.qt_pack_int4(Qt.data_ptr(), R, K, _ptr(col_src), packed.data_ptr(), _stream()))
     return packed
+
+
+def pack_stacked_enabled() -> bool:
+    return os.environ.get("QT_PACK_STACKED", "1") != "0"
+
+
+def pack_int4_stacked(Qt: torch.Tensor, segments, scale: Optional[torch.Tensor] = None):
+    lib = load()
+    _req(Qt, torch.int8, "Qt", 2)
+    K, R = Qt.shape
+    if not Qt.is_contiguous():
+        raise ValueError("Qt must be contiguous [K, R_total]")
+    G = 0
+    if scale is not None:
+        _req(scale, torch.float32, "scale", 2)
+        G = scale.shape[1]
+        if scale.shape[0] != R or not scale.is_contiguous():
+            raise ValueError(f"scale must be contiguous [R_total = {R}, G], got {tuple(scale.shape)}")
+    n = len(segments)
+    if n == 0:
+        return []
+    out = []
+    row0s, nrows, sdts = (ctypes.c_int32 * n)(), (ctypes.c_int32 * n)(), (ctypes.c_int32 * n)()
+    cols, packs, souts = (ctypes.c_void_p * n)(), (ctypes.c_void_p * n)(), (ctypes.c_void_p * n)()
+    for i, (row0, rows, col_src, sdt) in enumerate(segments):
+        row0, rows = int(row0), int(rows)
+        if rows <= 0 or row0 < 0 or row0 + rows > R:
+            raise ValueError(f"segment {i}: rows [{row0}, {row0 + rows}) outside the {R} stacked rows")
+        if col_src is not None:
+            _req(col_src, torch.int32, "col_src", 1)
+            if col_src.numel() != K or not col_src.is_contiguous():
+                raise ValueError("col_src must be contiguous int32 [K]")
+        packed = torch.empty((rows, (K + 7) // 8), dtype=torch.int32, device=Qt.device)
+        ws = None
+        if sdt is not None:
+            if scale is None:
+                raise ValueError("a segment asks for its scales but no scale table was given")
+            ws = torch.empty((rows, G), dtype=sdt, device=Qt.device)
+            sdts[i] = _dtype_code(ws)
+        row0s[i], nrows[i] = row0, rows
+        cols[i], packs[i], souts[i] = _ptr(col_src), packed.data_ptr(), _ptr(ws)
+        out.append((packed, ws))
+    check("qt_pack_int4_stacked", lib.qt_pack_int4_stacked(
+        Qt.data_ptr(), R, K, _ptr(scale), G, n, ctypes.cast(row0s, ctypes.c_void_p), ctypes.cast(nrows, ctypes.c_void_p),
+        ctypes.cast(cols, ctypes.c_void_p), ctypes.cast(packs, ctypes.c_void_p), ctypes.cast(souts, ctypes.c_void_p),
+        ctypes.cast(sdts, ctypes.c_void_p), _stream()))
+    return out
 
 
 def dequantize(Qt: torch.Tensor, scale: torch.Tensor, zp: torch.Tensor, g_of_col: torch.Tensor,
```

Measured after the change: 3.293 billion (median of 6 runs). Within noise of the previous version (+0.7%).
